# yukara-ikemiya/friendly-stable-audio-tools

Measured on NVIDIA B200. Metric: denoise_steps_per_s, higher is better.
Workload: dtype fp16 operands, fp32 accumulate (the reference's autocast dtype)

## Files before the change

### friendly-stable-audio-tools_b200/csrc/api.cu

```cuda
#include "../../include/satb200.h"
#include "common.cuh"
#include "gemm.cuh"
#include "kernels.h"

using namespace satb;

extern "C" {

int satb_snake_beta(const float* x, const float* alpha, const float* beta, float* y, int B, int C, long long T,
                    int logscale, void* stream) {
  SATB_REQUIRE(x && alpha && beta && y, "null argument");
  return launch_snake_beta(x, alpha, beta, y, B, C, T, logscale, static_cast<cudaStream_t>(stream));
}

int satb_layernorm(const float* x, const float* gamma, const float* beta, void* out16, int rows, int D, int bf16,
                   void* stream) {
  SATB_REQUIRE(x && gamma && out16, "null argument");
  return launch_layernorm(x, gamma, beta, out16, rows, D, nullptr, nullptr, 0, 1, 1, bf16 != 0,
                          static_cast<cudaStream_t>(stream));
}

int satb_linear_f32out(const void* a16, const void* w16, float* c, int M, int N, int K, int bf16, void* stream) {
  SATB_REQUIRE(a16 && w16 && c, "null argument");
  SATB_REQUIRE(M >= 1 && N >= 32 && N % 32 == 0 && K >= 8 && K % 8 == 0, "linear: need N % 32 == 0 and K % 8 == 0");
  CUtensorMap ta, tb;
  cudaStream_t st = static_cast<cudaStream_t>(stream);
  GemmShape s;
  s.L = M; s.batches = 1; s.N = N; s.K = K; s.n_taps = 1; s.tap_base = 0; s.tap_step = 0; s.b_tap_rows = N; s.stride = 1;
  EpiStore32::Params ep{c, N, nullptr};
  SATB_PROPAGATE(make_tmap_a(&ta, a16, K, M, 1, K, static_cast<int64_t>(M) * K));
  if ((N % 256 == 0 || N > 256) && gemm_use_2cta() && M >= 1024) {
    SATB_PROPAGATE(make_tmap_b(&tb, w16, K, N, K, 128));
    return bf16 ? launch_gemm_2cta<EpiStore32, 256, true>(ta, tb, s, ep, st) : launch_gemm_2cta<EpiStore32, 256, false>(ta, tb, s, ep, st);
  }
  if (N % 256 == 0 || N > 256) {
    SATB_PROPAGATE(make_tmap_b(&tb, w16, K, N, K, 256));
    return bf16 ? launch_gemm<EpiStore32, 256, true>(ta, tb, s, ep, st) : launch_gemm<EpiStore32, 256, false>(ta, tb, s, ep, st);
  } else if (N > 64) {
    SATB_PROPAGATE(make_tmap_b(&tb, w16, K, N, K, 128));
    return bf16 ? launch_gemm<EpiStore32, 128, true>(ta, tb, s, ep, st) : launch_gemm<EpiStore32, 128, false>(ta, tb, s, ep, st);
  }
  SATB_PROPAGATE(make_tmap_b(&tb, w16, K, N, K, 64));
  return bf16 ? launch_gemm<EpiStore32, 64, true>(ta, tb, s, ep, st) : launch_gemm<EpiStore32, 64, false>(ta, tb, s, ep, st);
}

int satb_sampler_update(const float* x, const float* v, const float* den_1, const float* den_2, const float* noise,
                        float* den, float* x_next, float* x_in_next, long long n, float c_skip, float c_out, float a,
                        float b, float c, float d, float s, float c_in_next, void* stream) {
  SATB_REQUIRE(x && v && den && x_next, "null argument");
  return launch_sampler_update(x, v, den_1, den_2, noise, den, x_next, x_in_next, n, c_skip, c_out, a, b, c, d, s,
                               c_in_next, static_cast<cudaStream_t>(stream));
}

int satb_attention(const void* q16, const void* k16, const void* v16, void* o16, int B, int H, int Hkv, int Nq, int Nk,
                   int bf16, void* stream) {
  SATB_REQUIRE(q16 && k16 && v16 && o16, "null argument");
  const int64_t dq = static_cast<int64_t>(H) * 64, dk = static_cast<int64_t>(Hkv) * 64;
  return launch_attention_tc(q16, k16, v16, o16, dq, dk, dk, dq, Nq * dq, Nk * dk, Nk * dk, Nq * dq, static_cast<int>(dq),
                             static_cast<int>(dk), static_cast<int>(dk), 0, 0, 0, B, H, Hkv, Nq, Nk, bf16 != 0,
                             static_cast<cudaStream_t>(stream));
}

int satb_debug_attention_occupancy(int dyn_smem, int carveout_pct) { return debug_attention_occupancy(dyn_smem, carveout_pct); }

int satb_attention_trace(const void* q16, const void* k16, const void* v16, void* o16, int B, int H, int Hkv, int Nq,
                         int Nk, int bf16, unsigned long long* dbg, void* stream) {
  const int64_t dq = static_cast<int64_t>(H) * 64, dk = static_cast<int64_t>(Hkv) * 64;
  return launch_attention_tc(q16, k16, v16, o16, dq, dk, dk, dq, Nq * dq, Nk * dk, Nk * dk, Nq * dq, static_cast<int>(dq),
                             static_cast<int>(dk), static_cast<int>(dk), 0, 0, 0, B, H, Hkv, Nq, Nk, bf16 != 0,
                             static_cast<cudaStream_t>(stream), dbg);
}

}
```

### friendly-stable-audio-tools_b200/csrc/dit.cu

```cuda
#include <cmath>
#include <cstring>
#include <map>
#include <string>
#include <tuple>
#include <vector>

#include "../../include/satb200.h"
#include "common.cuh"
#include "gemm.cuh"
#include "kernels.h"

namespace satb {

struct DevBuf {
  void* p = nullptr;
  size_t bytes = 0;
  int ensure(size_t need) {
    if (need <= bytes) return 0;
    if (p) cudaFree(p);
    p = nullptr;
    bytes = 0;
    cudaError_t e = cudaMalloc(&p, need);
    if (e != cudaSuccess) {
      set_last_error(std::string("cudaMalloc failed: ") + cudaGetErrorString(e) + " (" + std::to_string(need) + " B)");
      return -2;
    }
    bytes = need;
    return 0;
  }
  void release() {
    if (p) cudaFree(p);
    p = nullptr;
    bytes = 0;
  }
  template <class T>
  T* as() const {
    return static_cast<T*>(p);
  }
};

struct TmapCache {
  typedef std::tuple<const void*, int, int, int, int64_t, int64_t, int> Key;
  std::map<Key, CUtensorMap> maps;
  int get_a(const void* ptr, int K, int L, int batches, int64_t rs, int64_t bs, const CUtensorMap** out) {
    Key k(ptr, K, L, batches, rs, bs, -1);
    auto it = maps.find(k);
    if (it == maps.end()) {
      CUtensorMap m;
      SATB_PROPAGATE(make_tmap_a(&m, ptr, K, L, batches, rs, bs));
      it = maps.emplace(k, m).first;
    }
    *out = &it->second;
    return 0;
  }
  int get_b(const void* ptr, int K, int rows, int64_t rs, int box_rows, const CUtensorMap** out) {
    Key k(ptr, K, rows, 0, rs, 0, box_rows);
    auto it = maps.find(k);
    if (it == maps.end()) {
      CUtensorMap m;
      SATB_PROPAGATE(make_tmap_b(&m, ptr, K, rows, rs, box_rows));
      it = maps.emplace(k, m).first;
    }
    *out = &it->second;
    return 0;
  }
};

template <class Epi, int BN, bool BF16>
static int linear(TmapCache& tc, const void* A, int64_t lda, int M, int K, const void* W, int N,
                  const typename Epi::Params& ep, cudaStream_t stream) {
  const CUtensorMap *ta, *tb;
  SATB_PROPAGATE(tc.get_a(A, K, M, 1, lda, static_cast<int64_t>(M) * lda, &ta));
  GemmShape s;
  s.L = M; s.batches = 1; s.N = N; s.K = K; s.n_taps = 1; s.tap_base = 0; s.tap_step = 0; s.b_tap_rows = N; s.stride = 1;
  s.b_static = 1;
  if constexpr (BN == 256 || BN == 128) {
    if (gemm_use_2cta() && M >= 1024) {
      SATB_PROPAGATE(tc.get_b(W, K, N, K, BN / 2, &tb));
      return launch_gemm_2cta<Epi, BN, BF16>(*ta, *tb, s, ep, stream);
    }
  }
  SATB_PROPAGATE(tc.get_b(W, K, N, K, BN, &tb));
  return launch_gemm<Epi, BN, BF16>(*ta, *tb, s, ep, stream);
}

template <class Epi, bool BF16>
static int linear_auto(TmapCache& tc, const void* A, int64_t lda, int M, int K, const void* W, int N,
                       const typename Epi::Params& ep, cudaStream_t stream) {
  const double sms = device_sm_count();
  auto eff = [&](int bn) {
    const double waves = static_cast<double>(ceil_div(M, kBlockM)) * ceil_div(N, bn) / sms;
    return waves / std::ceil(waves);
  };
  if (N % 128 == 0 && eff(128) * 0.9 > eff(256)) return linear<Epi, 128, BF16>(tc, A, lda, M, K, W, N, ep, stream);
  return linear<Epi, 256, BF16>(tc, A, lda, M, K, W, N, ep, stream);
}

struct LayerW {
  float *pre_g = nullptr, *pre_b = nullptr, *ca_g = nullptr, *ca_b = nullptr, *ff_g = nullptr, *ff_b = nullptr;
  uint16_t *w_qkv = nullptr, *w_o = nullptr, *w_q = nullptr, *w_kv = nullptr, *w_co = nullptr, *w_ff1 = nullptr,
           *w_ff2 = nullptr;
  float *b_ff1 = nullptr, *b_ff2 = nullptr;
  float *c_qkv = nullptr, *d_qkv = nullptr, *c_q = nullptr, *d_q = nullptr, *c_ff1 = nullptr, *d_ff1 = nullptr;
};

}

using namespace satb;

struct SatbDit {
  SatbDitConfig cfg;
  int D, H, dh, C, Cin, ct, ce, gd, ge, ffi, depth, F, nf;
  int pdim = 0;
  float *pe0_w = nullptr, *pe2_w = nullptr;
  int Pp = 0;
  DevBuf ws_prep;
  bool bf16, adaln, qk_norm = false;
  bool ln_fused = false;
  int P;
  std::vector<LayerW> layers;
  std::vector<void*> owned;
  float *ts_w = nullptr, *te0_w = nullptr, *te0_b = nullptr, *te2_w = nullptr, *te2_b = nullptr;
  uint16_t *ce0_w = nullptr, *ce2_w = nullptr;
  float *ge0_w = nullptr, *ge2_w = nullptr;
  float *pre_w = nullptr, *post_w = nullptr, *pin_w = nullptr, *pout_w = nullptr, *inv_freq = nullptr;
  uint16_t *w_in16 = nullptr, *w_out16 = nullptr;
  float* w_ssg = nullptr;
  int* ff_perm = nullptr;
  std::map<std::string, int> loaded;
  bool finalized = false;
  int B = 0, Mctx = 0, Rc = 0;
  bool cfg_on = false, has_cross = false, has_global = false;
  TmapCache tmaps;
  DevBuf ws_h, ws_a16, ws_qkv, ws_attn, ws_q16, ws_ff, ws_ain, ws_y, ws_small, ws_cond, ws_kv, ws_rope, ws_stats;
  int rope_len = 0;
  int res_R = 0, res_L = 0, res_P = -1;
  bool prof_on = false;
  struct ProfRec { int cat; cudaEvent_t a, b; };
  std::vector<ProfRec> prof_recs;
  std::vector<cudaEvent_t> prof_pool;
  cudaEvent_t prof_event() {
    if (!prof_pool.empty()) { cudaEvent_t e = prof_pool.back(); prof_pool.pop_back(); return e; }
    cudaEvent_t e; cudaEventCreate(&e); return e;
  }

  template <class T>
  int alloc(T** p, size_t n) {
    void* q = nullptr;
    cudaError_t e = cudaMalloc(&q, n * sizeof(T) < 256 ? 256 : n * sizeof(T));
    if (e != cudaSuccess) {
      set_last_error(std::string("cudaMalloc failed: ") + cudaGetErrorString(e));
      return -2;
    }
    owned.push_back(q);
    *p = static_cast<T*>(q);
    return 0;
  }
};

static bool ends_with(const std::string& s, const std::string& suf) {
  return s.size() >= suf.size() && s.compare(s.size() - suf.size(), suf.size(), suf) == 0;
}

extern "C" {

const char* satb_last_error(void) { return get_last_error(); }
unsigned long long satb_launch_count(void) { return g_launch_count; }
void satb_reset_launch_count(void) { g_launch_count = 0; }
void satb_add_launch_count(unsigned long long n) { g_launch_count += n; }
int satb_abi_version(void) { return SATB_ABI_VERSION; }

int satb_dit_create(const SatbDitConfig* cfg, SatbDit** out) {
  SATB_REQUIRE(cfg && out, "null argument");
  SATB_REQUIRE(cfg->embed_dim % 128 == 0, "embed_dim must be a multiple of 128");
  SATB_REQUIRE(cfg->num_heads > 0 && cfg->embed_dim / cfg->num_heads == 64 && cfg->embed_dim % cfg->num_heads == 0,
               "head dim must be 64");
  SATB_REQUIRE(cfg->io_channels % 8 == 0 && cfg->io_channels % 32 == 0, "io_channels must be a multiple of 32");
  SATB_REQUIRE(cfg->patch_size == 1, "patch_size 1 only");
  SATB_REQUIRE(cfg->input_concat_dim >= 0 && cfg->input_concat_dim % 8 == 0, "input_concat_dim must be a multiple of 8");
  SATB_REQUIRE(cfg->prepend_cond_dim >= 0 && cfg->prepend_cond_dim % 4 == 0, "prepend_cond_dim must be a multiple of 4");
  SATB_REQUIRE(!(cfg->prepend_cond_dim > 0 && cfg->global_cond_type == 1),
               "prepend conditioning is supported with global_cond_type \"prepend\" only");
  SatbDit* d = new SatbDit();
  d->cfg = *cfg;
  d->D = cfg->embed_dim;
  d->H = cfg->num_heads;
  d->dh = d->D / d->H;
  d->C = cfg->io_channels;
  d->Cin = cfg->io_channels + (cfg->input_concat_dim > 0 ? cfg->input_concat_dim : 0);
  d->pdim = cfg->prepend_cond_dim > 0 ? cfg->prepend_cond_dim : 0;
  d->ct = cfg->cond_token_dim;
  d->ce = cfg->project_cond_tokens ? d->D : d->ct;
  d->gd = cfg->global_cond_dim;
  d->ge = cfg->project_global_cond ? d->D : d->gd;
  d->ffi = 4 * d->D;
  d->depth = cfg->depth;
  d->F = 128;
  const int rot = d->dh / 2 > 32 ? d->dh / 2 : 32;
  d->nf = rot / 2;
  d->bf16 = cfg->operand_dtype == 1;
  d->adaln = cfg->global_cond_type == 1;
  d->qk_norm = cfg->qk_norm != 0;
  d->P = d->adaln ? 0 : 1;
  if (d->ct > 0) {
    if (d->ce % 64 != 0 || d->H % (d->ce / 64) != 0) {
      delete d;
      set_last_error("cond embed dim must be a multiple of 64 with kv heads dividing num_heads");
      return -1;
    }
  }
  if (d->gd > 0 && d->ge != d->D) {
    delete d;
    set_last_error("global embed dim must equal embed_dim");
    return -1;
  }
  SATB_REQUIRE(d->nf == 16, "rotary dim must be 32 (head dim 64)");
  d->layers.resize(d->depth);
  *out = d;
  return 0;
}

void satb_dit_destroy(SatbDit* d) {
  if (!d) return;
  for (void* p : d->owned) cudaFree(p);
  d->ws_h.release(); d->ws_a16.release(); d->ws_qkv.release(); d->ws_attn.release(); d->ws_q16.release();
  d->ws_ff.release(); d->ws_ain.release(); d->ws_y.release(); d->ws_small.release(); d->ws_cond.release();
  d->ws_kv.release(); d->ws_rope.release(); d->ws_stats.release(); d->ws_prep.release();
  delete d;
}

int satb_dit_load_weight(SatbDit* d, const char* name_c, const float* src, long long numel, void* stream_v) {
  SATB_REQUIRE(d && name_c && src, "null argument");
  cudaStream_t st = static_cast<cudaStream_t>(stream_v);
  const std::string name(name_c);
  const int D = d->D, C = d->C, Cin = d->Cin;
  auto copy_f32 = [&](float** dst, long long expect) -> int {
    SATB_REQUIRE(numel == expect, ("bad size for " + name).c_str());
    if (!*dst) SATB_PROPAGATE(d->alloc(dst, expect));
    SATB_CHECK_CUDA(cudaMemcpyAsync(*dst, src, expect * sizeof(float), cudaMemcpyDeviceToDevice, st));
    return 0;
  };
  auto cast16 = [&](uint16_t** dst, int rows, int cols, const int* perm) -> int {
    SATB_REQUIRE(numel == static_cast<long long>(rows) * cols, ("bad size for " + name).c_str());
    if (!*dst) SATB_PROPAGATE(d->alloc(dst, static_cast<size_t>(rows) * cols));
    return launch_cast_rows(src, *dst, perm, rows, cols, cols, cols, d->bf16, st);
  };
  d->finalized = false;
  d->loaded[name] = 1;
  if (name == "timestep_features.weight") return copy_f32(&d->ts_w, d->F);
  if (name == "to_timestep_embed.0.weight") return copy_f32(&d->te0_w, static_cast<long long>(D) * 2 * d->F);
  if (name == "to_timestep_embed.0.bias") return copy_f32(&d->te0_b, D);
  if (name == "to_timestep_embed.2.weight") return copy_f32(&d->te2_w, static_cast<long long>(D) * D);
  if (name == "to_timestep_embed.2.bias") return copy_f32(&d->te2_b, D);
  if (name == "to_cond_embed.0.weight") return cast16(&d->ce0_w, d->ce, d->ct, nullptr);
  if (name == "to_cond_embed.2.weight") return cast16(&d->ce2_w, d->ce, d->ce, nullptr);
  if (name == "to_global_embed.0.weight") return copy_f32(&d->ge0_w, static_cast<long long>(d->ge) * d->gd);
  if (name == "to_global_embed.2.weight") return copy_f32(&d->ge2_w, static_cast<long long>(d->ge) * d->ge);
  if (name == "preprocess_conv.weight") return copy_f32(&d->pre_w, static_cast<long long>(Cin) * Cin);
  if (name == "to_prepend_embed.0.weight" && d->pdim > 0) return copy_f32(&d->pe0_w, static_cast<long long>(D) * d->pdim);
  if (name == "to_prepend_embed.2.weight" && d->pdim > 0) return copy_f32(&d->pe2_w, static_cast<long long>(D) * D);
  if (name == "postprocess_conv.weight") return copy_f32(&d->post_w, static_cast<long long>(C) * C);
  if (name == "transformer.project_in.weight") return copy_f32(&d->pin_w, static_cast<long long>(D) * Cin);
  if (name == "transformer.project_out.weight") return copy_f32(&d->pout_w, static_cast<long long>(C) * D);
  if (name == "transformer.rotary_pos_emb.inv_freq") return copy_f32(&d->inv_freq, d->nf);
  const std::string lp = "transformer.layers.";
  if (name.compare(0, lp.size(), lp) == 0) {
    const size_t dot = name.find('.', lp.size());
    SATB_REQUIRE(dot != std::string::npos, ("bad key " + name).c_str());
    const int li = atoi(name.substr(lp.size(), dot - lp.size()).c_str());
    SATB_REQUIRE(li >= 0 && li < d->depth, ("layer index out of range in " + name).c_str());
    LayerW& L = d->layers[li];
    const std::string k = name.substr(dot + 1);
    if (k == "pre_norm.gamma") return copy_f32(&L.pre_g, D);
    if (k == "pre_norm.beta") return copy_f32(&L.pre_b, D);
    if (k == "cross_attend_norm.gamma") return copy_f32(&L.ca_g, D);
    if (k == "cross_attend_norm.beta") return copy_f32(&L.ca_b, D);
    if (k == "ff_norm.gamma") return copy_f32(&L.ff_g, D);
    if (k == "ff_norm.beta") return copy_f32(&L.ff_b, D);
    if (k == "self_attn.to_qkv.weight") return cast16(&L.w_qkv, 3 * D, D, nullptr);
    if (k == "self_attn.to_out.weight") return cast16(&L.w_o, D, D, nullptr);
    if (k == "cross_attn.to_q.weight") return cast16(&L.w_q, D, D, nullptr);
    if (k == "cross_attn.to_kv.weight") return cast16(&L.w_kv, 2 * d->ce, d->ce, nullptr);
    if (k == "cross_attn.to_out.weight") return cast16(&L.w_co, D, D, nullptr);
    if (k == "ff.ff.0.proj.weight" || k == "ff.ff.0.proj.bias") {
      if (!d->ff_perm) {
        std::vector<int> perm(2 * d->ffi);
        for (int n = 0; n < 2 * d->ffi; ++n) {
          const int g = n / 64, w = n % 64;
          perm[n] = w < 32 ? g * 32 + w : d->ffi + g * 32 + (w - 32);
        }
        SATB_PROPAGATE(d->alloc(&d->ff_perm, perm.size()));
        SATB_CHECK_CUDA(cudaMemcpy(d->ff_perm, perm.data(), perm.size() * sizeof(int), cudaMemcpyHostToDevice));
      }
      if (ends_with(k, "weight")) return cast16(&L.w_ff1, 2 * d->ffi, D, d->ff_perm);
      SATB_REQUIRE(numel == 2 * d->ffi, ("bad size for " + name).c_str());
      if (!L.b_ff1) SATB_PROPAGATE(d->alloc(&L.b_ff1, 2 * d->ffi));
      return launch_gather_f32(src, L.b_ff1, d->ff_perm, 2 * d->ffi, st);
    }
    if (k == "ff.ff.2.weight") return cast16(&L.w_ff2, D, d->ffi, nullptr);
    if (k == "ff.ff.2.bias") return copy_f32(&L.b_ff2, D);
    if (k == "to_scale_shift_gate.1.weight") {
      SATB_REQUIRE(numel == 6LL * D * D, ("bad size for " + name).c_str());
      if (!d->w_ssg) SATB_PROPAGATE(d->alloc(&d->w_ssg, static_cast<size_t>(d->depth) * 6 * D * D));
      SATB_CHECK_CUDA(cudaMemcpyAsync(d->w_ssg + static_cast<size_t>(li) * 6 * D * D, src, numel * sizeof(float),
                                      cudaMemcpyDeviceToDevice, st));
      return 0;
    }
  }
  d->loaded.erase(name);
  set_last_error("unknown DiT weight key: " + name);
  return -4;
}

int satb_dit_finalize(SatbDit* d, void* stream_v) {
  SATB_REQUIRE(d, "null handle");
  cudaStream_t st = static_cast<cudaStream_t>(stream_v);
  const int D = d->D, C = d->C;
  SATB_REQUIRE(d->ts_w && d->te0_w && d->te0_b && d->te2_w && d->te2_b, "timestep embedding weights missing");
  SATB_REQUIRE(d->pin_w && d->pout_w && d->pre_w && d->post_w, "project_in/out or pre/post conv weights missing");
  SATB_REQUIRE(d->inv_freq, "rotary inv_freq missing");
  if (d->ct > 0) SATB_REQUIRE(d->ce0_w && d->ce2_w, "to_cond_embed weights missing");
  if (d->gd > 0) SATB_REQUIRE(d->ge0_w && d->ge2_w, "to_global_embed weights missing");
  for (int i = 0; i < d->depth; ++i) {
    const LayerW& L = d->layers[i];
    SATB_REQUIRE(L.pre_g && L.ff_g && L.w_qkv && L.w_o && L.w_ff1 && L.w_ff2, "transformer layer weights missing");
    if (d->ct > 0) SATB_REQUIRE(L.ca_g && L.w_q && L.w_kv && L.w_co, "cross-attention weights missing");
  }
  if (d->adaln) SATB_REQUIRE(d->w_ssg, "adaLN to_scale_shift_gate weights missing");
  SATB_CHECK_CUDA(cudaStreamSynchronize(st));
  const int Cin = d->Cin;
  if (d->pdim > 0) SATB_REQUIRE(d->pe0_w && d->pe2_w, "to_prepend_embed weights missing");
  std::vector<float> pin(static_cast<size_t>(D) * Cin), pout(static_cast<size_t>(C) * D), pre(Cin * Cin), post(C * C);
  SATB_CHECK_CUDA(cudaMemcpy(pin.data(), d->pin_w, pin.size() * 4, cudaMemcpyDeviceToHost));
  SATB_CHECK_CUDA(cudaMemcpy(pout.data(), d->pout_w, pout.size() * 4, cudaMemcpyDeviceToHost));
  SATB_CHECK_CUDA(cudaMemcpy(pre.data(), d->pre_w, pre.size() * 4, cudaMemcpyDeviceToHost));
  SATB_CHECK_CUDA(cudaMemcpy(post.data(), d->post_w, post.size() * 4, cudaMemcpyDeviceToHost));
  std::vector<float> fin(static_cast<size_t>(D) * Cin), fout(static_cast<size_t>(C) * D);
  for (int n = 0; n < D; ++n)
    for (int c = 0; c < Cin; ++c) {
      double acc = pin[static_cast<size_t>(n) * Cin + c];
      for (int j = 0; j < Cin; ++j) acc += static_cast<double>(pin[static_cast<size_t>(n) * Cin + j]) * pre[j * Cin + c];
      fin[static_cast<size_t>(n) * Cin + c] = static_cast<float>(acc);
    }
  for (int c = 0; c < C; ++c)
    for (int k = 0; k < D; ++k) {
      double acc = pout[static_cast<size_t>(c) * D + k];
      for (int j = 0; j < C; ++j) acc += static_cast<double>(post[c * C + j]) * pout[static_cast<size_t>(j) * D + k];
      fout[static_cast<size_t>(c) * D + k] = static_cast<float>(acc);
    }
  float *tmp_in = nullptr, *tmp_out = nullptr;
  SATB_CHECK_CUDA(cudaMalloc(&tmp_in, fin.size() * 4));
  SATB_CHECK_CUDA(cudaMalloc(&tmp_out, fout.size() * 4));
  SATB_CHECK_CUDA(cudaMemcpy(tmp_in, fin.data(), fin.size() * 4, cudaMemcpyHostToDevice));
  SATB_CHECK_CUDA(cudaMemcpy(tmp_out, fout.data(), fout.size() * 4, cudaMemcpyHostToDevice));
  if (!d->w_in16) SATB_PROPAGATE(d->alloc(&d->w_in16, fin.size()));
  if (!d->w_out16) SATB_PROPAGATE(d->alloc(&d->w_out16, fout.size()));
  int rc = launch_cast_rows(tmp_in, d->w_in16, nullptr, D, Cin, Cin, Cin, d->bf16, st);
  if (rc == 0) rc = launch_cast_rows(tmp_out, d->w_out16, nullptr, C, D, D, D, d->bf16, st);
  cudaStreamSynchronize(st);
  cudaFree(tmp_in);
  cudaFree(tmp_out);
  SATB_PROPAGATE(rc);
  d->ln_fused = !d->adaln && !d->qk_norm && ln_fold_enabled() && d->D == 6 * 256;
  if (d->ln_fused) {
    for (int i = 0; i < d->depth; ++i) {
      LayerW& L = d->layers[i];
      auto prep = [&](float** c, float** dd, const uint16_t* w, const float* g, const float* b, int rows) -> int {
        bool has_beta = false;
        if (b) {
          std::vector<float> hb(D);
          SATB_CHECK_CUDA(cudaMemcpy(hb.data(), b, D * sizeof(float), cudaMemcpyDeviceToHost));
          for (float v : hb) has_beta = has_beta || v != 0.f;
        }
        if (!*c) SATB_PROPAGATE(d->alloc(c, rows));
        float* scratch = nullptr;
        if (has_beta && !*dd) SATB_PROPAGATE(d->alloc(dd, rows));
        if (!has_beta) {
          *dd = nullptr;
          SATB_PROPAGATE(d->alloc(&scratch, rows));
        }
        return launch_ln_fold_vectors(w, g, has_beta ? b : nullptr, *c, has_beta ? *dd : scratch, rows, D, d->bf16, st);
      };
      SATB_PROPAGATE(prep(&L.c_qkv, &L.d_qkv, L.w_qkv, L.pre_g, L.pre_b, 3 * D));
      if (d->ct > 0) SATB_PROPAGATE(prep(&L.c_q, &L.d_q, L.w_q, L.ca_g, L.ca_b, D));
      SATB_PROPAGATE(prep(&L.c_ff1, &L.d_ff1, L.w_ff1, L.ff_g, L.ff_b, 2 * d->ffi));
    }
    SATB_CHECK_CUDA(cudaStreamSynchronize(st));
  }
  d->tmaps.maps.clear();
  d->finalized = true;
  return 0;
}

}

static int ensure_rope(SatbDit* d, int N_seq) {
  if (d->rope_len == N_seq) return 0;
  std::vector<float> inv(d->nf), tab(static_cast<size_t>(2) * N_seq * d->nf);
  SATB_CHECK_CUDA(cudaMemcpy(inv.data(), d->inv_freq, d->nf * 4, cudaMemcpyDeviceToHost));
  for (int p = 0; p < N_seq; ++p)
    for (int j = 0; j < d->nf; ++j) {
      const float f = static_cast<float>(p) * inv[j];
      tab[static_cast<size_t>(p) * d->nf + j] = cosf(f);
      tab[static_cast<size_t>(N_seq) * d->nf + static_cast<size_t>(p) * d->nf + j] = sinf(f);
    }
  SATB_PROPAGATE(d->ws_rope.ensure(tab.size() * 4));
  SATB_CHECK_CUDA(cudaMemcpy(d->ws_rope.p, tab.data(), tab.size() * 4, cudaMemcpyHostToDevice));
  d->rope_len = N_seq;
  return 0;
}

extern "C" {

int satb_dit_reserve(SatbDit* d, int R, int L) {
  SATB_REQUIRE(d && d->finalized, "weights not finalized");
  SATB_REQUIRE(R >= 1 && L >= 1, "bad shape");
  const int N_seq = L + d->P;
  const size_t M = static_cast<size_t>(R) * N_seq;
  const int D = d->D;
  SATB_PROPAGATE(d->ws_h.ensure(M * D * 4));
  SATB_PROPAGATE(d->ws_a16.ensure(M * D * 2));
  SATB_PROPAGATE(d->ws_qkv.ensure(M * 3 * D * 2));
  SATB_PROPAGATE(d->ws_attn.ensure(M * D * 2));
  SATB_PROPAGATE(d->ws_q16.ensure(M * D * 2));
  SATB_PROPAGATE(d->ws_ff.ensure(M * d->ffi * 2));
  SATB_PROPAGATE(d->ws_ain.ensure(M * d->Cin * 2));
  SATB_PROPAGATE(d->ws_y.ensure(M * d->C * 4));
  SATB_PROPAGATE(d->ws_stats.ensure(3 * M * kLnSlots * sizeof(float2)));
  SATB_PROPAGATE(ensure_rope(d, N_seq));
  d->tmaps.maps.clear();
  d->res_R = R;
  d->res_L = L;
  d->res_P = d->P;
  return 0;
}

}

struct SmallWs {
  float *fourier, *te_h, *tok, *ge_h, *ge, *ssg;
};
static SmallWs small_ws(SatbDit* d, int R) {
  SmallWs s;
  float* p = d->ws_small.as<float>();
  s.fourier = p; p += static_cast<size_t>(R) * 2 * d->F;
  s.te_h = p;    p += static_cast<size_t>(R) * d->D;
  s.tok = p;     p += static_cast<size_t>(R) * d->D;
  s.ge_h = p;    p += static_cast<size_t>(R) * d->D;
  s.ge = p;      p += static_cast<size_t>(R) * d->D;
  s.ssg = p;
  return s;
}

extern "C" {

int satb_dit_set_prepend_cond(SatbDit* d, const float* prepend, int B, int n_tokens, void* stream_v) {
  SATB_REQUIRE(d && d->finalized, "weights not finalized");
  cudaStream_t st = static_cast<cudaStream_t>(stream_v);
  if (!prepend || n_tokens <= 0) {
    d->Pp = 0;
    d->P = d->adaln ? 0 : 1;
    return 0;
  }
  SATB_REQUIRE(d->pdim > 0 && !d->adaln, "this model has no prepend conditioning");
  SATB_REQUIRE(B >= 1, "bad batch");
  const size_t rows = static_cast<size_t>(B) * n_tokens;
  SATB_REQUIRE(rows <= 4096, "too many prepend tokens");
  SATB_PROPAGATE(d->ws_prep.ensure(2 * rows * d->D * sizeof(float)));
  float* emb = d->ws_prep.as<float>();
  float* hid = emb + rows * d->D;
  SATB_PROPAGATE(launch_skinny_linear(prepend, d->pe0_w, nullptr, nullptr, hid, static_cast<int>(rows), d->pdim, d->D, 1, st));
  SATB_PROPAGATE(launch_skinny_linear(hid, d->pe2_w, nullptr, nullptr, emb, static_cast<int>(rows), d->D, d->D, 0, st));
  d->Pp = n_tokens;
  d->P = 1 + n_tokens;
  return 0;
}

int satb_dit_prepare_cond(SatbDit* d, const float* cross, const float* neg_cross, const float* global, int B, int Mctx,
                          int use_cfg, void* stream_v) {
  SATB_REQUIRE(d && d->finalized, "weights not finalized");
  SATB_REQUIRE(B >= 1, "bad batch");
  cudaStream_t st = static_cast<cudaStream_t>(stream_v);
  const int D = d->D;
  d->B = B;
  d->cfg_on = use_cfg != 0;
  d->has_cross = cross != nullptr && d->ct > 0;
  d->has_global = global != nullptr && d->gd > 0;
  d->Mctx = d->has_cross ? Mctx : 0;
  d->Rc = d->has_cross ? ((d->cfg_on && neg_cross) ? 2 * B : B) : 0;
  SATB_REQUIRE(!(neg_cross && !d->cfg_on), "negative conditioning requires CFG");
  SATB_PROPAGATE(d->ws_small.ensure(static_cast<size_t>(2 * B) * (2 * d->F + 4 * D + 6 * D * d->depth) * 4 + 4096));
  SmallWs sw = small_ws(d, 2 * B);
  if (d->has_global) {
    SATB_PROPAGATE(launch_skinny_linear(global, d->ge0_w, nullptr, nullptr, sw.ge_h, B, d->gd, d->ge, 1, st));
    SATB_PROPAGATE(launch_skinny_linear(sw.ge_h, d->ge2_w, nullptr, nullptr, sw.ge, B, d->ge, d->ge, 0, st));
  }
  if (d->has_cross) {
    SATB_REQUIRE(Mctx >= 1, "empty cross-attention context");
    const size_t rows = static_cast<size_t>(d->Rc) * Mctx;
    const size_t in_b = rows * d->ct * 2, mid_b = rows * d->ce * 2;
    SATB_PROPAGATE(d->ws_cond.ensure(in_b + 2 * mid_b + 1024));
    uint16_t* in16 = d->ws_cond.as<uint16_t>();
    uint16_t* mid16 = in16 + rows * d->ct;
    uint16_t* ce16 = mid16 + rows * d->ce;
    SATB_PROPAGATE(launch_cast_rows(cross, in16, nullptr, B * Mctx, d->ct, d->ct, d->ct, d->bf16, st));
    if (d->Rc == 2 * B)
      SATB_PROPAGATE(launch_cast_rows(neg_cross, in16 + static_cast<size_t>(B) * Mctx * d->ct, nullptr, B * Mctx,
                                      d->ct, d->ct, d->ct, d->bf16, st));
    SATB_PROPAGATE(d->ws_kv.ensure(static_cast<size_t>(d->depth) * rows * 2 * d->ce * 2));
    d->tmaps.maps.clear();
    const int Mr = static_cast<int>(rows);
    if (d->bf16) {
      typedef EpiStore16<true> E;
      SATB_PROPAGATE((linear<E, 128, true>(d->tmaps, in16, d->ct, Mr, d->ct, d->ce0_w, d->ce, E::Params{mid16, d->ce, nullptr, 1}, st)));
      SATB_PROPAGATE((linear<E, 128, true>(d->tmaps, mid16, d->ce, Mr, d->ce, d->ce2_w, d->ce, E::Params{ce16, d->ce, nullptr, 0}, st)));
      for (int i = 0; i < d->depth; ++i) {
        uint16_t* kv = d->ws_kv.as<uint16_t>() + static_cast<size_t>(i) * rows * 2 * d->ce;
        if (d->qk_norm) {
          typedef EpiHeadNorm16<true> EN;
          SATB_PROPAGATE((linear<EN, 128, true>(d->tmaps, ce16, d->ce, Mr, d->ce, d->layers[i].w_kv, 2 * d->ce,
                                                 EN::Params{kv, 2 * d->ce, d->ce, 0, 1, nullptr, nullptr}, st)));
        } else {
          SATB_PROPAGATE((linear<E, 128, true>(d->tmaps, ce16, d->ce, Mr, d->ce, d->layers[i].w_kv, 2 * d->ce, E::Params{kv, 2 * d->ce, nullptr, 0}, st)));
        }
      }
    } else {
      typedef EpiStore16<false> E;
      SATB_PROPAGATE((linear<E, 128, false>(d->tmaps, in16, d->ct, Mr, d->ct, d->ce0_w, d->ce, E::Params{mid16, d->ce, nullptr, 1}, st)));
      SATB_PROPAGATE((linear<E, 128, false>(d->tmaps, mid16, d->ce, Mr, d->ce, d->ce2_w, d->ce, E::Params{ce16, d->ce, nullptr, 0}, st)));
      for (int i = 0; i < d->depth; ++i) {
        uint16_t* kv = d->ws_kv.as<uint16_t>() + static_cast<size_t>(i) * rows * 2 * d->ce;
        if (d->qk_norm) {
          typedef EpiHeadNorm16<false> EN;
          SATB_PROPAGATE((linear<EN, 128, false>(d->tmaps, ce16, d->ce, Mr, d->ce, d->layers[i].w_kv, 2 * d->ce,
                                                 EN::Params{kv, 2 * d->ce, d->ce, 0, 1, nullptr, nullptr}, st)));
        } else {
          SATB_PROPAGATE((linear<E, 128, false>(d->tmaps, ce16, d->ce, Mr, d->ce, d->layers[i].w_kv, 2 * d->ce, E::Params{kv, 2 * d->ce, nullptr, 0}, st)));
        }
      }
    }
  }
  return 0;
}

}

struct ProfScope {
  SatbDit* d; int cat; cudaStream_t st; cudaEvent_t a = nullptr, b = nullptr;
  ProfScope(SatbDit* d_, int cat_, cudaStream_t st_) : d(d_), cat(cat_), st(st_) {
    if (d->prof_on) { a = d->prof_event(); b = d->prof_event(); cudaEventRecord(a, st); }
  }
  ~ProfScope() {
    if (a) { cudaEventRecord(b, st); d->prof_recs.push_back({cat, a, b}); }
  }
};
enum { PROF_FF_IN = 0, PROF_FF_OUT, PROF_QKV, PROF_ATTN_SELF, PROF_ATTN_OUT, PROF_CROSS, PROF_LN, PROF_OTHER, PROF_NCAT };

template <bool BF16>
static int dit_forward_impl(SatbDit* d, const float* x, const float* t, float* out, int B, int L, float cfg_scale,
                            float scale_phi, cudaStream_t st, float* hidden_out) {
  const int D = d->D, C = d->C, H = d->H, P = d->P;
  const int R = d->cfg_on ? 2 * B : B;
  const int N_seq = L + P;
  const int M = R * N_seq;
  const int Mc = d->Rc * N_seq;
  SmallWs sw = small_ws(d, 2 * d->B);
  float* h = d->ws_h.as<float>();
  uint16_t* a16 = d->ws_a16.as<uint16_t>();
  uint16_t* qkv = d->ws_qkv.as<uint16_t>();
  uint16_t* att = d->ws_attn.as<uint16_t>();
  uint16_t* q16 = d->ws_q16.as<uint16_t>();
  uint16_t* ff = d->ws_ff.as<uint16_t>();
  uint16_t* ain = d->ws_ain.as<uint16_t>();
  float* y = d->ws_y.as<float>();
  const float* cos_tab = d->ws_rope.as<float>();
  const float* sin_tab = cos_tab + static_cast<size_t>(N_seq) * d->nf;

  SATB_PROPAGATE(launch_fourier(t, d->ts_w, sw.fourier, B, d->F, st));
  SATB_PROPAGATE(launch_skinny_linear(sw.fourier, d->te0_w, d->te0_b, nullptr, sw.te_h, B, 2 * d->F, D, 1, st));
  SATB_PROPAGATE(launch_skinny_linear(sw.te_h, d->te2_w, d->te2_b, d->has_global ? sw.ge : nullptr, sw.tok, B, D, D,
                                      d->adaln ? 1 : 0, st));
  SATB_PROPAGATE(launch_dit_pre(x, ain, R, B, d->Cin, L, P, BF16, st));
  SATB_PROPAGATE((linear<EpiStore32, 256, BF16>(d->tmaps, ain, d->Cin, M, d->Cin, d->w_in16, D, EpiStore32::Params{h, D, nullptr}, st)));
  const int64_t ssg_ld = static_cast<int64_t>(d->depth) * 6 * D;
  if (P > 0) {
    SATB_PROPAGATE(launch_write_prepend(sw.tok, d->Pp > 0 ? d->ws_prep.as<float>() : nullptr, h, R, B, N_seq, D, d->Pp, st));
  } else {
    SATB_PROPAGATE(launch_skinny_linear(sw.tok, d->w_ssg, nullptr, nullptr, sw.ssg, B, D, d->depth * 6 * D, 0, st));
    SATB_PROPAGATE(launch_gate_sigmoid(sw.ssg, B, d->depth, D, st));
  }

  const bool fused = d->ln_fused;
  float2* S1 = d->ws_stats.as<float2>();
  float2* S2 = S1 + static_cast<size_t>(M) * kLnSlots;
  float2* S3 = S2 + static_cast<size_t>(M) * kLnSlots;
  auto fold = [&](const float2* st_, const float* c, const float* dd) {
    return LnFold{st_, c, dd, 1.0f / static_cast<float>(D), 1e-5f, kLnSlots};
  };
  const LnFold no_ln{nullptr, nullptr, nullptr, 0.f, 0.f, 0};
  for (int i = 0; i < d->depth; ++i) {
    const LayerW& W = d->layers[i];
    const float* ssg_l = d->adaln ? sw.ssg + static_cast<size_t>(i) * 6 * D : nullptr;
    if (!fused || i == 0) {
      ProfScope ps(d, PROF_LN, st);
      SATB_PROPAGATE(launch_layernorm(h, W.pre_g, W.pre_b, a16, M, D, ssg_l, ssg_l ? ssg_l + D : nullptr, ssg_ld, N_seq, B, BF16, st));
    }
    {
      ProfScope ps(d, PROF_QKV, st);
      if (d->qk_norm) {
        typedef EpiHeadNorm16<BF16> E;
        typename E::Params ep{qkv, 3 * D, 2 * D, 2 * D, N_seq, cos_tab, sin_tab};
        SATB_PROPAGATE((linear<E, 256, BF16>(d->tmaps, a16, D, M, D, W.w_qkv, 3 * D, ep, st)));
      } else {
        if (fused && i > 0) {
          typedef EpiQkvRope<BF16, true> E;
          typename E::Params ep{qkv, 3 * D, 2 * D, N_seq, cos_tab, sin_tab, fold(S1, W.c_qkv, W.d_qkv)};
          SATB_PROPAGATE((linear<E, 256, BF16>(d->tmaps, a16, D, M, D, W.w_qkv, 3 * D, ep, st)));
        } else {
          typedef EpiQkvRope<BF16> E;
          typename E::Params ep{qkv, 3 * D, 2 * D, N_seq, cos_tab, sin_tab, no_ln};
          SATB_PROPAGATE((linear<E, 256, BF16>(d->tmaps, a16, D, M, D, W.w_qkv, 3 * D, ep, st)));
        }
      }
    }
    {
      ProfScope ps(d, PROF_ATTN_SELF, st);
      const int64_t qs = static_cast<int64_t>(N_seq) * 3 * D;
      SATB_PROPAGATE(launch_attention_tc(qkv, qkv, qkv, att, 3 * D, 3 * D, 3 * D, D, qs, qs, qs,
                                         static_cast<int64_t>(N_seq) * D, 3 * D, 3 * D, 3 * D, 0, D, 2 * D, R, H, H,
                                         N_seq, N_seq, BF16, st));
    }
    {
      ProfScope ps(d, PROF_ATTN_OUT, st);
      if (fused) {
        typedef EpiResidualLN<BF16> E;
        typename E::Params ep{h, D, nullptr, a16, W.ca_g, W.ff_g, S2, S3, Mc};
        SATB_PROPAGATE((linear<E, 256, BF16>(d->tmaps, att, D, M, D, W.w_o, D, ep, st)));
      } else {
        EpiResidual::Params ep{h, D, nullptr, ssg_l ? ssg_l + 2 * D : nullptr, N_seq, static_cast<int>(ssg_ld), B};
        SATB_PROPAGATE((linear_auto<EpiResidual, BF16>(d->tmaps, att, D, M, D, W.w_o, D, ep, st)));
      }
    }
    if (Mc > 0) {
      ProfScope ps(d, PROF_CROSS, st);
      const int Hkv = d->ce / 64;
      if (!fused) SATB_PROPAGATE(launch_layernorm(h, W.ca_g, W.ca_b, a16, Mc, D, nullptr, nullptr, 0, N_seq, 1, BF16, st));
      if (d->qk_norm) {
        typedef EpiHeadNorm16<BF16> E;
        typename E::Params ep{q16, D, D, 0, N_seq, nullptr, nullptr};
        SATB_PROPAGATE((linear_auto<E, BF16>(d->tmaps, a16, D, Mc, D, W.w_q, D, ep, st)));
      } else {
        if (fused) {
          typedef EpiStore16<BF16, true> E;
          typename E::Params ep{q16, D, nullptr, 0, fold(S2, W.c_q, W.d_q)};
          SATB_PROPAGATE((linear_auto<E, BF16>(d->tmaps, a16, D, Mc, D, W.w_q, D, ep, st)));
        } else {
          typedef EpiStore16<BF16> E;
          typename E::Params ep{q16, D, nullptr, 0, no_ln};
          SATB_PROPAGATE((linear_auto<E, BF16>(d->tmaps, a16, D, Mc, D, W.w_q, D, ep, st)));
        }
      }
      const uint16_t* kv = d->ws_kv.as<uint16_t>() + static_cast<size_t>(i) * d->Rc * d->Mctx * 2 * d->ce;
      const int64_t kvs = static_cast<int64_t>(d->Mctx) * 2 * d->ce;
      SATB_PROPAGATE(launch_attention_tc(q16, kv, kv, att, D, 2 * d->ce, 2 * d->ce, D, static_cast<int64_t>(N_seq) * D,
                                         kvs, kvs, static_cast<int64_t>(N_seq) * D, D, 2 * d->ce, 2 * d->ce, 0, 0,
                                         d->ce, d->Rc, H, Hkv, N_seq, d->Mctx, BF16, st));
      if (fused) {
        typedef EpiResidualLN<BF16> E;
        typename E::Params ep{h, D, nullptr, a16, W.ff_g, W.ff_g, S3, S3, Mc};
        SATB_PROPAGATE((linear<E, 256, BF16>(d->tmaps, att, D, Mc, D, W.w_co, D, ep, st)));
      } else {
        EpiResidual::Params ep{h, D, nullptr, nullptr, N_seq, 0, 1};
        SATB_PROPAGATE((linear_auto<EpiResidual, BF16>(d->tmaps, att, D, Mc, D, W.w_co, D, ep, st)));
      }
    }
    if (!fused) {
      ProfScope ps(d, PROF_LN, st);
      SATB_PROPAGATE(launch_layernorm(h, W.ff_g, W.ff_b, a16, M, D, ssg_l ? ssg_l + 3 * D : nullptr,
                                      ssg_l ? ssg_l + 4 * D : nullptr, ssg_ld, N_seq, B, BF16, st));
    }
    {
      ProfScope ps(d, PROF_FF_IN, st);
      if (fused) {
        typedef EpiSwiglu<BF16, true> E;
        typename E::Params ep{ff, d->ffi, W.b_ff1, fold(S3, W.c_ff1, W.d_ff1)};
        SATB_PROPAGATE((linear<E, 256, BF16>(d->tmaps, a16, D, M, D, W.w_ff1, 2 * d->ffi, ep, st)));
      } else {
        typedef EpiSwiglu<BF16> E;
        typename E::Params ep{ff, d->ffi, W.b_ff1, no_ln};
        SATB_PROPAGATE((linear<E, 256, BF16>(d->tmaps, a16, D, M, D, W.w_ff1, 2 * d->ffi, ep, st)));
      }
    }
    {
      ProfScope ps(d, PROF_FF_OUT, st);
      if (fused) {
        const bool last = i + 1 == d->depth;
        typedef EpiResidualLN<BF16> E;
        typename E::Params ep{h, D, W.b_ff2, a16, last ? nullptr : d->layers[i + 1].pre_g, nullptr, last ? nullptr : S1, nullptr, M};
        SATB_PROPAGATE((linear<E, 256, BF16>(d->tmaps, ff, d->ffi, M, d->ffi, W.w_ff2, D, ep, st)));
      } else {
        EpiResidual::Params ep{h, D, W.b_ff2, ssg_l ? ssg_l + 5 * D : nullptr, N_seq, static_cast<int>(ssg_ld), B};
        SATB_PROPAGATE((linear_auto<EpiResidual, BF16>(d->tmaps, ff, d->ffi, M, d->ffi, W.w_ff2, D, ep, st)));
      }
    }
  }
  if (hidden_out)
    SATB_CHECK_CUDA(cudaMemcpyAsync(hidden_out, h, static_cast<size_t>(M) * D * 4, cudaMemcpyDeviceToDevice, st));
  if (!fused || d->depth == 0) SATB_PROPAGATE(launch_cast_rows(h, a16, nullptr, M, D, D, D, BF16, st));
  SATB_PROPAGATE((linear<EpiStore32, 64, BF16>(d->tmaps, a16, D, M, D, d->w_out16, C, EpiStore32::Params{y, C, nullptr}, st)));
  SATB_PROPAGATE(launch_dit_post(y, out, B, C, L, N_seq, P, d->cfg_on ? 1 : 0, cfg_scale, scale_phi, st));
  return 0;
}

extern "C" {

int satb_dit_forward(SatbDit* d, const float* x, const float* t, float* out, int B, int L, float cfg_scale,
                     float scale_phi, void* stream_v) {
  SATB_REQUIRE(d && d->finalized, "weights not finalized");
  SATB_REQUIRE(B == d->B, "batch size differs from satb_dit_prepare_cond");
  const int R = d->cfg_on ? 2 * B : B;
  if (R > d->res_R || L != d->res_L || d->P != d->res_P) SATB_PROPAGATE(satb_dit_reserve(d, R, L));
  cudaStream_t st = static_cast<cudaStream_t>(stream_v);
  return d->bf16 ? dit_forward_impl<true>(d, x, t, out, B, L, cfg_scale, scale_phi, st, nullptr)
                 : dit_forward_impl<false>(d, x, t, out, B, L, cfg_scale, scale_phi, st, nullptr);
}

int satb_dit_profile(SatbDit* d, int enable) {
  SATB_REQUIRE(d, "null handle");
  d->prof_on = enable != 0;
  return 0;
}
int satb_dit_profile_read(SatbDit* d, float* ms, int* count) {
  SATB_REQUIRE(d && ms && count, "null argument");
  for (int i = 0; i < PROF_NCAT; ++i) { ms[i] = 0.f; count[i] = 0; }
  for (auto& r : d->prof_recs) {
    SATB_CHECK_CUDA(cudaEventSynchronize(r.b));
    float t = 0.f;
    SATB_CHECK_CUDA(cudaEventElapsedTime(&t, r.a, r.b));
    ms[r.cat] += t;
    count[r.cat] += 1;
    d->prof_pool.push_back(r.a);
    d->prof_pool.push_back(r.b);
  }
  d->prof_recs.clear();
  return 0;
}

int satb_dit_forward_debug(SatbDit* d, const float* x, const float* t, float* out, float* hidden, int B, int L,
                           float cfg_scale, float scale_phi, void* stream_v) {
  SATB_REQUIRE(d && d->finalized, "weights not finalized");
  SATB_REQUIRE(B == d->B, "batch size differs from satb_dit_prepare_cond");
  const int R = d->cfg_on ? 2 * B : B;
  if (R > d->res_R || L != d->res_L || d->P != d->res_P) SATB_PROPAGATE(satb_dit_reserve(d, R, L));
  cudaStream_t st = static_cast<cudaStream_t>(stream_v);
  return d->bf16 ? dit_forward_impl<true>(d, x, t, out, B, L, cfg_scale, scale_phi, st, hidden)
                 : dit_forward_impl<false>(d, x, t, out, B, L, cfg_scale, scale_phi, st, hidden);
}

}
```

### friendly-stable-audio-tools_b200/csrc/gemm.cuh

```cuda
#pragma once
#include <type_traits>

#include "common.cuh"
#include "ptx.cuh"

namespace satb {

__device__ __forceinline__ int split_part(int idx, int n_parts) { return n_parts == 3 ? (idx == 2 ? 0 : idx + 1) : idx; }

struct GemmShape {
  int L;
  int batches;
  int N;
  int K;
  int n_taps;
  int tap_base;
  int tap_step;
  int b_tap_rows;
  int stride;
  int b_static = 0;
  int n_parts = 1;
  int b_part_rows = 0;
};

constexpr int kBlockM = 128;
constexpr int kBlockK = 64;
constexpr int kUmmaK = 16;
constexpr int kGemmThreads = 384;
constexpr int kSmemBudget = 220 * 1024;

constexpr int kEpiWarps = 8;
template <int BN, int kEpiStage = 0>
struct GemmCfg {
  static constexpr int kStageA = kBlockM * kBlockK * 2;
  static constexpr int kStageB = BN * kBlockK * 2;
  static constexpr int kStage = kStageA + kStageB;
  static constexpr int kAvail = kSmemBudget - 1024 - kEpiWarps * kEpiStage;
  static constexpr int kStages = kAvail / kStage > 8 ? 8 : kAvail / kStage;
  static constexpr int kTmemCols = 2 * BN < 32 ? 32 : 2 * BN;
  static constexpr int kSmemBytes = kStages * kStage + 1024  + 256  + kEpiWarps * kEpiStage;
  static_assert(BN == 64 || BN == 128 || BN == 256, "BN must be 64/128/256");
};

struct EpiCtx {
  int row;
  int l;
  int batch;
  int col0;
  bool valid;
  int l0;
  int L;
  int lane;
  float* stage;
  int n_tile;
  int half;
};

template <class E, class = void>
struct EpiHasState : std::false_type {};
template <class E>
struct EpiHasState<E, std::void_t<typename E::State>> : std::true_type {};
struct EpiNoStateHolder {
  struct State {};
};
template <class Epi>
struct EpiTile {
  using State = typename std::conditional<EpiHasState<Epi>::value, Epi, EpiNoStateHolder>::type::State;
  template <int N>
  __device__ static __forceinline__ void apply(const typename Epi::Params& p, const EpiCtx& c, const uint32_t (&r)[N], State& st) {
    if constexpr (EpiHasState<Epi>::value) Epi::apply(p, c, r, st);
    else Epi::apply(p, c, r);
  }
  __device__ static __forceinline__ void begin(const typename Epi::Params& p, const EpiCtx& c, State& st) {
    if constexpr (EpiHasState<Epi>::value) Epi::tile_begin(p, c, st);
  }
  __device__ static __forceinline__ void end(const typename Epi::Params& p, const EpiCtx& c, State& st) {
    if constexpr (EpiHasState<Epi>::value) Epi::tile_end(p, c, st);
  }
};

template <class Epi, int BN, bool BF16>
__global__ void __launch_bounds__(kGemmThreads, 1)
gemm_tcgen05_kernel(const __grid_constant__ CUtensorMap tmA, const __grid_constant__ CUtensorMap tmB,
                    const __grid_constant__ CUtensorMap tmA2, const GemmShape s, const typename Epi::Params ep) {
  using Cfg = GemmCfg<BN, Epi::kStageBytes>;
  extern __shared__ uint8_t smem_raw[];
  uint8_t* smem = reinterpret_cast<uint8_t*>((reinterpret_cast<uintptr_t>(smem_raw) + 1023) & ~uintptr_t(1023));
  uint64_t* bars = reinterpret_cast<uint64_t*>(smem + Cfg::kStages * Cfg::kStage);
  uint64_t* full_bar = bars;
  uint64_t* empty_bar = bars + Cfg::kStages;
  uint64_t* tfull_bar = bars + 2 * Cfg::kStages;
  uint64_t* tempty_bar = tfull_bar + 2;
  uint32_t* tmem_slot = reinterpret_cast<uint32_t*>(tempty_bar + 2);

  const int warp = threadIdx.x >> 5;
  const int lane = threadIdx.x & 31;

  const int m_tiles = (s.L + kBlockM - 1) / kBlockM;
  const int n_tiles = (s.N + BN - 1) / BN;
  const int tiles_per_n = m_tiles * s.batches;
  const int total_tiles = tiles_per_n * n_tiles;
  const int kb_per_tap = (s.K + kBlockK - 1) / kBlockK;
  const int kb_per_part = kb_per_tap * s.n_taps;
  const int num_kb = kb_per_part * s.n_parts;

  if (threadIdx.x == 0) {
    tma_prefetch_desc(&tmA);
    tma_prefetch_desc(&tmB);
    for (int i = 0; i < Cfg::kStages; ++i) {
      mbar_init(&full_bar[i], 1);
      mbar_init(&empty_bar[i], 1);
    }
    for (int i = 0; i < 2; ++i) {
      mbar_init(&tfull_bar[i], 1);
      mbar_init(&tempty_bar[i], 8);
    }
    fence_mbar_init();
  }
  if (warp == 2) {
    tmem_alloc(tmem_slot, Cfg::kTmemCols);
    tmem_relinquish();
  }
  tc_fence_before();
  __syncthreads();
  tc_fence_after();
  const uint32_t tmem_base = *tmem_slot;
  pdl_launch_dependents();
  const bool is_producer_warp = warp == 0;
  if (!is_producer_warp) pdl_wait();

  if (warp == 0) {
    if (elect_one()) {
      int pre = 0;
      if (s.b_static && static_cast<int>(blockIdx.x) < total_tiles) {
        pre = num_kb < Cfg::kStages ? num_kb : Cfg::kStages;
        const int n0 = (static_cast<int>(blockIdx.x) / tiles_per_n) * BN;
        for (int kb = 0; kb < pre; ++kb) {
          const int pidx = kb / kb_per_part, kbp = kb - pidx * kb_per_part;
          const int part = split_part(pidx, s.n_parts);
          const int tap = kbp / kb_per_tap;
          const int k0 = (kbp - tap * kb_per_tap) * kBlockK;
          mbar_expect_tx(&full_bar[kb], Cfg::kStage);
          tma_load_2d(smem + kb * Cfg::kStage + Cfg::kStageA, &tmB, &full_bar[kb], k0,
                      tap * s.b_tap_rows + n0 + (part == 2 ? s.b_part_rows : 0));
        }
      }
      pdl_wait();
      int stage = 0;
      uint32_t phase = 0;
      for (int tile = blockIdx.x; tile < total_tiles; tile += gridDim.x) {
        const int nt = tile / tiles_per_n;
        const int rem = tile - nt * tiles_per_n;
        const int batch = rem / m_tiles;
        const int m0 = (rem - batch * m_tiles) * kBlockM;
        const int n0 = nt * BN;
        for (int kb = 0; kb < num_kb; ++kb) {
          const int pidx = kb / kb_per_part, kbp = kb - pidx * kb_per_part;
          const int part = split_part(pidx, s.n_parts);
          const int tap = kbp / kb_per_tap;
          const int k0 = (kbp - tap * kb_per_tap) * kBlockK;
          mbar_wait(&empty_bar[stage], phase ^ 1);
          uint8_t* sa = smem + stage * Cfg::kStage;
          uint8_t* sb = sa + Cfg::kStageA;
          const bool b_done = tile == static_cast<int>(blockIdx.x) && kb < pre;
          if (!b_done) mbar_expect_tx(&full_bar[stage], Cfg::kStage);
          const int u = s.tap_base + tap * s.tap_step;
          int ph = 0, ro = u;
          if (s.stride > 1) {
            ro = (u >= 0) ? u / s.stride : -((-u + s.stride - 1) / s.stride);
            ph = u - ro * s.stride;
          }
          tma_load_4d(sa, part == 1 ? &tmA2 : &tmA, &full_bar[stage], k0, ph, m0 + ro, batch);
          if (!b_done)
            tma_load_2d(sb, &tmB, &full_bar[stage], k0, tap * s.b_tap_rows + n0 + (part == 2 ? s.b_part_rows : 0));
          if (++stage == Cfg::kStages) {
            stage = 0;
            phase ^= 1;
          }
        }
      }
    }
  } else if (warp == 1) {
    if (elect_one()) {
      constexpr uint32_t idesc = make_idesc_f16(kBlockM, BN, BF16);
      int stage = 0;
      uint32_t phase = 0;
      int acc = 0;
      uint32_t acc_phase = 0;
      for (int tile = blockIdx.x; tile < total_tiles; tile += gridDim.x) {
        mbar_wait(&tempty_bar[acc], acc_phase ^ 1);
        tc_fence_after();
        const uint32_t d_tmem = tmem_base + acc * BN;
        for (int kb = 0; kb < num_kb; ++kb) {
          mbar_wait(&full_bar[stage], phase);
          tc_fence_after();
          const uint32_t a_addr = smem_u32(smem + stage * Cfg::kStage);
          const uint32_t b_addr = a_addr + Cfg::kStageA;
#pragma unroll
          for (int k = 0; k < kBlockK / kUmmaK; ++k) {
            const uint64_t da = make_desc_kmajor_sw128(a_addr + k * kUmmaK * 2);
            const uint64_t db = make_desc_kmajor_sw128(b_addr + k * kUmmaK * 2);
            umma_f16_ss(d_tmem, da, db, idesc, (kb | k) != 0 ? 1u : 0u);
          }
          umma_commit(&empty_bar[stage]);
          if (++stage == Cfg::kStages) {
            stage = 0;
            phase ^= 1;
          }
        }
        umma_commit(&tfull_bar[acc]);
        if (++acc == 2) {
          acc = 0;
          acc_phase ^= 1;
        }
      }
    }
  } else if (warp >= 4) {
    const int q = warp & 3;
    const int half = (warp - 4) >> 2;
    constexpr int kChunks = BN / Epi::kCols;
    int acc = 0;
    uint32_t acc_phase = 0;
    for (int tile = blockIdx.x; tile < total_tiles; tile += gridDim.x) {
      const int nt = tile / tiles_per_n;
      const int rem = tile - nt * tiles_per_n;
      const int batch = rem / m_tiles;
      const int m0 = (rem - batch * m_tiles) * kBlockM;
      const int n0 = nt * BN;
      mbar_wait(&tfull_bar[acc], acc_phase);
      tc_fence_after();
      EpiCtx c;
      c.l = m0 + q * 32 + lane;
      c.batch = batch;
      c.row = batch * s.L + c.l;
      c.valid = c.l < s.L;
      c.l0 = m0 + q * 32;
      c.L = s.L;
      c.lane = lane;
      c.n_tile = nt;
      c.half = half;
      c.stage = Epi::kStageBytes > 0
                    ? reinterpret_cast<float*>(smem + Cfg::kStages * Cfg::kStage + 256 + (warp - 4) * Epi::kStageBytes)
                    : nullptr;
      const uint32_t t_row = tmem_base + (static_cast<uint32_t>(q * 32) << 16) + acc * BN;
      int n_valid = (s.N - n0 + Epi::kCols - 1) / Epi::kCols;
      if (n_valid > kChunks) n_valid = kChunks;
      uint32_t r0[Epi::kCols], r1[Epi::kCols];
      auto load_chunk = [&](int ci, uint32_t (&dst)[Epi::kCols]) {
#pragma unroll
        for (int j = 0; j < Epi::kCols / 32; ++j) {
          uint32_t(&rj)[32] = *reinterpret_cast<uint32_t(*)[32]>(&dst[j * 32]);
          tmem_ld_32x32(t_row + ci * Epi::kCols + j * 32, rj);
        }
      };
      typename EpiTile<Epi>::State est;
      EpiTile<Epi>::begin(ep, c, est);
      if (half < n_valid) {
        load_chunk(half, r0);
        tmem_ld_wait();
      }
#pragma unroll 1
      for (int ci = half; ci < n_valid; ci += 4) {
        const bool has1 = ci + 2 < n_valid;
        if (has1) load_chunk(ci + 2, r1);
        c.col0 = n0 + ci * Epi::kCols;
        EpiTile<Epi>::apply(ep, c, r0, est);
        tmem_ld_wait();
        if (has1) {
          if (ci + 4 < n_valid) load_chunk(ci + 4, r0);
          c.col0 = n0 + (ci + 2) * Epi::kCols;
          EpiTile<Epi>::apply(ep, c, r1, est);
          tmem_ld_wait();
        }
      }
      EpiTile<Epi>::end(ep, c, est);
      tc_fence_before();
      __syncwarp();
      if (lane == 0) mbar_arrive(&tempty_bar[acc]);
      if (++acc == 2) {
        acc = 0;
        acc_phase ^= 1;
      }
    }
  }
  tc_fence_before();
  __syncthreads();
  if (warp == 2) {
    tc_fence_after();
    tmem_dealloc(tmem_base, Cfg::kTmemCols);
  }
}

template <int BN, int kEpiStage = 0>
struct Gemm2Cfg {
  static constexpr int kStageA = kBlockM * kBlockK * 2;
  static constexpr int kStageB = (BN / 2) * kBlockK * 2;
  static constexpr int kStage = kStageA + kStageB;
  static constexpr int kAvail = kSmemBudget - 1024 - kEpiWarps * kEpiStage;
  static constexpr int kStages = kAvail / kStage > 8 ? 8 : kAvail / kStage;
  static constexpr int kTmemCols = 2 * BN;
  static constexpr int kSmemBytes = kStages * kStage + 1024 + 256 + kEpiWarps * kEpiStage;
  static_assert(BN == 256 || BN == 128, "BN must be 128/256");
};

template <class Epi, int BN, bool BF16>
__global__ void __cluster_dims__(2, 1, 1) __launch_bounds__(kGemmThreads, 1)
gemm_tcgen05_2cta_kernel(const __grid_constant__ CUtensorMap tmA, const __grid_constant__ CUtensorMap tmB,
                         const __grid_constant__ CUtensorMap tmA2, const GemmShape s, const typename Epi::Params ep) {
  using Cfg = Gemm2Cfg<BN, Epi::kStageBytes>;
  extern __shared__ uint8_t smem_raw[];
  uint8_t* smem = reinterpret_cast<uint8_t*>((reinterpret_cast<uintptr_t>(smem_raw) + 1023) & ~uintptr_t(1023));
  uint64_t* bars = reinterpret_cast<uint64_t*>(smem + Cfg::kStages * Cfg::kStage);
  uint64_t* full_bar = bars;
  uint64_t* empty_bar = bars + Cfg::kStages;
  uint64_t* tfull_bar = bars + 2 * Cfg::kStages;
  uint64_t* tempty_bar = tfull_bar + 2;
  uint32_t* tmem_slot = reinterpret_cast<uint32_t*>(tempty_bar + 2);

  const int warp = threadIdx.x >> 5;
  const int lane = threadIdx.x & 31;
  const uint32_t rank = cluster_ctarank();
  const int cluster_id = blockIdx.x >> 1, n_clusters = gridDim.x >> 1;

  const int m_tiles = (s.L + 2 * kBlockM - 1) / (2 * kBlockM);
  const int n_tiles = (s.N + BN - 1) / BN;
  const int tiles_per_n = m_tiles * s.batches;
  const int total_tiles = tiles_per_n * n_tiles;
  const int kb_per_tap = (s.K + kBlockK - 1) / kBlockK;
  const int kb_per_part = kb_per_tap * s.n_taps;
  const int num_kb = kb_per_part * s.n_parts;

  if (threadIdx.x == 0) {
    tma_prefetch_desc(&tmA);
    tma_prefetch_desc(&tmB);
    for (int i = 0; i < Cfg::kStages; ++i) {
      mbar_init(&full_bar[i], 1);
      mbar_init(&empty_bar[i], 1);
    }
    for (int i = 0; i < 2; ++i) {
      mbar_init(&tfull_bar[i], 1);
      mbar_init(&tempty_bar[i], 16);
    }
    fence_mbar_init();
  }
  cluster_sync_all();
  if (warp == 2) {
    tmem_alloc_2sm(tmem_slot, Cfg::kTmemCols);
    tmem_relinquish_2sm();
  }
  tc_fence_before();
  __syncthreads();
  tc_fence_after();
  const uint32_t tmem_base = *tmem_slot;
  pdl_launch_dependents();
  if (warp != 0) pdl_wait();

  if (warp == 0) {
    if (elect_one()) {
      int pre = 0;
      if (s.b_static && cluster_id < total_tiles) {
        pre = num_kb < Cfg::kStages ? num_kb : Cfg::kStages;
        const int n0 = (cluster_id / tiles_per_n) * BN + rank * (BN / 2);
        for (int kb = 0; kb < pre; ++kb) {
          const int pidx = kb / kb_per_part, kbp = kb - pidx * kb_per_part;
          const int part = split_part(pidx, s.n_parts);
          const int tap = kbp / kb_per_tap;
          const int k0 = (kbp - tap * kb_per_tap) * kBlockK;
          if (rank == 0) mbar_expect_tx(&full_bar[kb], 2 * Cfg::kStage);
          tma_load_2d_2sm(smem + kb * Cfg::kStage + Cfg::kStageA, &tmB, &full_bar[kb], k0,
                          tap * s.b_tap_rows + n0 + (part == 2 ? s.b_part_rows : 0));
        }
      }
      pdl_wait();
      int stage = 0;
      uint32_t phase = 0;
      for (int tile = cluster_id; tile < total_tiles; tile += n_clusters) {
        const int nt = tile / tiles_per_n;
        const int rem = tile - nt * tiles_per_n;
        const int batch = rem / m_tiles;
        const int m0 = (rem - batch * m_tiles) * 2 * kBlockM + rank * kBlockM;
        const int n0 = nt * BN + rank * (BN / 2);
        for (int kb = 0; kb < num_kb; ++kb) {
          const int pidx = kb / kb_per_part, kbp = kb - pidx * kb_per_part;
          const int part = split_part(pidx, s.n_parts);
          const int tap = kbp / kb_per_tap;
          const int k0 = (kbp - tap * kb_per_tap) * kBlockK;
          mbar_wait(&empty_bar[stage], phase ^ 1);
          uint8_t* sa = smem + stage * Cfg::kStage;
          uint8_t* sb = sa + Cfg::kStageA;
          const bool b_done = tile == cluster_id && kb < pre;
          if (rank == 0 && !b_done) mbar_expect_tx(&full_bar[stage], 2 * Cfg::kStage);
          const int u = s.tap_base + tap * s.tap_step;
          int ph = 0, ro = u;
          if (s.stride > 1) {
            ro = (u >= 0) ? u / s.stride : -((-u + s.stride - 1) / s.stride);
            ph = u - ro * s.stride;
          }
          tma_load_4d_2sm(sa, part == 1 ? &tmA2 : &tmA, &full_bar[stage], k0, ph, m0 + ro, batch);
          if (!b_done)
            tma_load_2d_2sm(sb, &tmB, &full_bar[stage], k0, tap * s.b_tap_rows + n0 + (part == 2 ? s.b_part_rows : 0));
          if (++stage == Cfg::kStages) {
            stage = 0;
            phase ^= 1;
          }
        }
      }
    }
  } else if (warp == 1) {
    if (rank == 0 && elect_one()) {
      constexpr uint32_t idesc = make_idesc_f16(2 * kBlockM, BN, BF16);
      int stage = 0;
      uint32_t phase = 0;
      int acc = 0;
      uint32_t acc_phase = 0;
      for (int tile = cluster_id; tile < total_tiles; tile += n_clusters) {
        mbar_wait(&tempty_bar[acc], acc_phase ^ 1);
        tc_fence_after();
        const uint32_t d_tmem = tmem_base + acc * BN;
        for (int kb = 0; kb < num_kb; ++kb) {
          mbar_wait(&full_bar[stage], phase);
          tc_fence_after();
          const uint32_t a_addr = smem_u32(smem + stage * Cfg::kStage);
          const uint32_t b_addr = a_addr + Cfg::kStageA;
#pragma unroll
          for (int k = 0; k < kBlockK / kUmmaK; ++k) {
            const uint64_t da = make_desc_kmajor_sw128(a_addr + k * kUmmaK * 2);
            const uint64_t db = make_desc_kmajor_sw128(b_addr + k * kUmmaK * 2);
            umma_f16_ss_2sm(d_tmem, da, db, idesc, (kb | k) != 0 ? 1u : 0u);
          }
          umma_commit_2sm(&empty_bar[stage]);
          if (++stage == Cfg::kStages) {
            stage = 0;
            phase ^= 1;
          }
        }
        umma_commit_2sm(&tfull_bar[acc]);
        if (++acc == 2) {
          acc = 0;
          acc_phase ^= 1;
        }
      }
    }
  } else if (warp >= 4) {
    const int q = warp & 3;
    const int half = (warp - 4) >> 2;
    constexpr int kChunks = BN / Epi::kCols;
    int acc = 0;
    uint32_t acc_phase = 0;
    for (int tile = cluster_id; tile < total_tiles; tile += n_clusters) {
      const int nt = tile / tiles_per_n;
      const int rem = tile - nt * tiles_per_n;
      const int batch = rem / m_tiles;
      const int m0 = (rem - batch * m_tiles) * 2 * kBlockM + rank * kBlockM;
      const int n0 = nt * BN;
      mbar_wait(&tfull_bar[acc], acc_phase);
      tc_fence_after();
      EpiCtx c;
      c.l = m0 + q * 32 + lane;
      c.batch = batch;
      c.row = batch * s.L + c.l;
      c.valid = c.l < s.L;
      c.l0 = m0 + q * 32;
      c.L = s.L;
      c.lane = lane;
      c.n_tile = nt;
      c.half = half;
      c.stage = Epi::kStageBytes > 0
                    ? reinterpret_cast<float*>(smem + Cfg::kStages * Cfg::kStage + 256 + (warp - 4) * Epi::kStageBytes)
                    : nullptr;
      const uint32_t t_row = tmem_base + (static_cast<uint32_t>(q * 32) << 16) + acc * BN;
      int n_valid = (s.N - n0 + Epi::kCols - 1) / Epi::kCols;
      if (n_valid > kChunks) n_valid = kChunks;
      uint32_t r0[Epi::kCols], r1[Epi::kCols];
      auto load_chunk = [&](int ci, uint32_t (&dst)[Epi::kCols]) {
#pragma unroll
        for (int j = 0; j < Epi::kCols / 32; ++j) {
          uint32_t(&rj)[32] = *reinterpret_cast<uint32_t(*)[32]>(&dst[j * 32]);
          tmem_ld_32x32(t_row + ci * Epi::kCols + j * 32, rj);
        }
      };
      typename EpiTile<Epi>::State est;
      EpiTile<Epi>::begin(ep, c, est);
      if (half < n_valid) {
        load_chunk(half, r0);
        tmem_ld_wait();
      }
#pragma unroll 1
      for (int ci = half; ci < n_valid; ci += 4) {
        const bool has1 = ci + 2 < n_valid;
        if (has1) load_chunk(ci + 2, r1);
        c.col0 = n0 + ci * Epi::kCols;
        EpiTile<Epi>::apply(ep, c, r0, est);
        tmem_ld_wait();
        if (has1) {
          if (ci + 4 < n_valid) load_chunk(ci + 4, r0);
          c.col0 = n0 + (ci + 2) * Epi::kCols;
          EpiTile<Epi>::apply(ep, c, r1, est);
          tmem_ld_wait();
        }
      }
      EpiTile<Epi>::end(ep, c, est);
      tc_fence_before();
      __syncwarp();
      if (lane == 0) mbar_arrive_remote(&tempty_bar[acc], 0);
      if (++acc == 2) {
        acc = 0;
        acc_phase ^= 1;
      }
    }
  }
  tc_fence_before();
  cluster_sync_all();
  if (warp == 2) {
    tc_fence_after();
    tmem_dealloc_2sm(tmem_base, Cfg::kTmemCols);
  }
}


constexpr int kLnSlots = 12;
struct LnFold {
  const float2* stats;
  const float* c;
  const float* d;
  float inv_dim;
  float eps;
  int n_slots;
};
struct LnRow {
  float rstd, mr;
};
__device__ __forceinline__ LnRow ln_row(const LnFold& f, int row) {
  const float4* sp = reinterpret_cast<const float4*>(f.stats + static_cast<size_t>(row) * kLnSlots);
  float s1 = 0.f, s2 = 0.f;
#pragma unroll
  for (int i = 0; i < kLnSlots / 2; ++i) {
    if (2 * i < f.n_slots) {
      const float4 v = __ldg(sp + i);
      s1 += v.x + v.z;
      s2 += v.y + v.w;
    }
  }
  const float mean = s1 * f.inv_dim;
  const float var = fmaxf(s2 * f.inv_dim - mean * mean, 0.f);
  LnRow r;
  r.rstd = rsqrtf(var + f.eps);
  r.mr = mean * r.rstd;
  return r;
}
__device__ __forceinline__ void ln_apply4(const LnFold& f, const LnRow& r, float& v0, float& v1, float& v2, float& v3, int col) {
  const float4 cc = __ldg(reinterpret_cast<const float4*>(f.c + col));
  v0 = fmaf(v0, r.rstd, -r.mr * cc.x);
  v1 = fmaf(v1, r.rstd, -r.mr * cc.y);
  v2 = fmaf(v2, r.rstd, -r.mr * cc.z);
  v3 = fmaf(v3, r.rstd, -r.mr * cc.w);
  if (f.d) {
    const float4 dd = __ldg(reinterpret_cast<const float4*>(f.d + col));
    v0 += dd.x; v1 += dd.y; v2 += dd.z; v3 += dd.w;
  }
}

__device__ __forceinline__ float silu_f(float x) { return x / (1.0f + __expf(-x)); }

template <bool BF16, bool LN = false>
struct EpiStore16 {
  static constexpr int kCols = 32;
  static constexpr int kStageBytes = 0;
  struct Params {
    void* out;
    int ld;
    const float* bias;
    int act;
    LnFold ln = LnFold{nullptr, nullptr, nullptr, 0.f, 0.f, 0};
  };
  __device__ static __forceinline__ void apply(const Params& p, const EpiCtx& c, const uint32_t (&r)[32]) {
    if (!c.valid) return;
    float v[32];
#pragma unroll
    for (int j = 0; j < 32; ++j) v[j] = __uint_as_float(r[j]);
    if constexpr (LN) {
      const LnRow lr = ln_row(p.ln, c.row);
#pragma unroll
      for (int j = 0; j < 32; j += 4) ln_apply4(p.ln, lr, v[j], v[j + 1], v[j + 2], v[j + 3], c.col0 + j);
    }
    if (p.bias) {
#pragma unroll
      for (int j = 0; j < 32; j += 4) {
        const float4 b = __ldg(reinterpret_cast<const float4*>(p.bias + c.col0 + j));
        v[j] += b.x; v[j + 1] += b.y; v[j + 2] += b.z; v[j + 3] += b.w;
      }
    }
    uint32_t o[16];
#pragma unroll
    for (int j = 0; j < 16; ++j) {
      float a = v[2 * j], b = v[2 * j + 1];
      if (p.act == 1) {
        a = silu_f(a);
        b = silu_f(b);
      }
      o[j] = Op16<BF16>::pack(a, b);
    }
    uint4* dst = reinterpret_cast<uint4*>(static_cast<uint16_t*>(p.out) + static_cast<size_t>(c.row) * p.ld + c.col0);
#pragma unroll
    for (int j = 0; j < 4; ++j) dst[j] = make_uint4(o[4 * j], o[4 * j + 1], o[4 * j + 2], o[4 * j + 3]);
  }
};

struct EpiStore32 {
  static constexpr int kCols = 32;
  static constexpr int kStageBytes = 0;
  struct Params {
    float* out;
    int ld;
    const float* bias;
  };
  __device__ static __forceinline__ void apply(const Params& p, const EpiCtx& c, const uint32_t (&r)[32]) {
    if (!c.valid) return;
    float4* dst = reinterpret_cast<float4*>(p.out + static_cast<size_t>(c.row) * p.ld + c.col0);
#pragma unroll
    for (int j = 0; j < 8; ++j) {
      float4 v = make_float4(__uint_as_float(r[4 * j]), __uint_as_float(r[4 * j + 1]), __uint_as_float(r[4 * j + 2]),
                             __uint_as_float(r[4 * j + 3]));
      if (p.bias) {
        const float4 b = __ldg(reinterpret_cast<const float4*>(p.bias + c.col0) + j);
        v.x += b.x; v.y += b.y; v.z += b.z; v.w += b.w;
      }
      dst[j] = v;
    }
  }
};

struct EpiResidual {
  static constexpr int kCols = 32;
  static constexpr int kStageBytes = 0;
  struct Params {
    float* h;
    int ld;
    const float* bias;
    const float* gate;
    int rows_per_item;
    int gate_ld;
    int n_items;
  };
  __device__ static __forceinline__ void apply(const Params& p, const EpiCtx& c, const uint32_t (&r)[32]) {
    if (!c.valid) return;
    float4* dst = reinterpret_cast<float4*>(p.h + static_cast<size_t>(c.row) * p.ld + c.col0);
    const float4* g = p.gate ? reinterpret_cast<const float4*>(
                                   p.gate + static_cast<size_t>((c.row / p.rows_per_item) % p.n_items) * p.gate_ld + c.col0)
                             : nullptr;
#pragma unroll
    for (int j = 0; j < 8; ++j) {
      float4 v = make_float4(__uint_as_float(r[4 * j]), __uint_as_float(r[4 * j + 1]), __uint_as_float(r[4 * j + 2]),
                             __uint_as_float(r[4 * j + 3]));
      if (p.bias) {
        const float4 b = __ldg(reinterpret_cast<const float4*>(p.bias + c.col0) + j);
        v.x += b.x; v.y += b.y; v.z += b.z; v.w += b.w;
      }
      if (g) {
        const float4 gg = __ldg(g + j);
        v.x *= gg.x; v.y *= gg.y; v.z *= gg.z; v.w *= gg.w;
      }
      asm volatile("red.global.add.v4.f32 [%0], {%1, %2, %3, %4};" ::"l"(dst + j), "f"(v.x), "f"(v.y), "f"(v.z), "f"(v.w)
                   : "memory");
    }
  }
};

template <bool BF16>
struct EpiResidualLN {
  static constexpr int kCols = 32;
  static constexpr int kStageBytes = 32 * 36 * 4;
  struct Params {
    float* h;
    int ld;
    const float* bias;
    void* x16;
    const float* gamma_lo;
    const float* gamma_hi;
    float2* stats_lo;
    float2* stats_hi;
    int split;
  };
  struct State {
    float s1[8], s2[8];
  };
  __device__ static __forceinline__ void tile_begin(const Params&, const EpiCtx&, State& st) {
#pragma unroll
    for (int i = 0; i < 8; ++i) st.s1[i] = st.s2[i] = 0.f;
  }
  __device__ static __forceinline__ void apply(const Params& p, const EpiCtx& c, const uint32_t (&r)[32], State& st) {
    const int g = c.lane & 7, r0 = c.lane >> 3;
    const int col = c.col0 + 4 * g;
    float4 old[8];
#pragma unroll
    for (int i = 0; i < 8; ++i) {
      const int l = c.l0 + r0 + 4 * i;
      old[i] = l < c.L ? *reinterpret_cast<const float4*>(p.h + (static_cast<size_t>(c.batch) * c.L + l) * p.ld + col)
                       : make_float4(0.f, 0.f, 0.f, 0.f);
    }
    float* stg = c.stage;
    {
      float4* mine = reinterpret_cast<float4*>(stg + c.lane * 36);
#pragma unroll
      for (int j = 0; j < 8; ++j)
        mine[j] = make_float4(__uint_as_float(r[4 * j]), __uint_as_float(r[4 * j + 1]), __uint_as_float(r[4 * j + 2]),
                              __uint_as_float(r[4 * j + 3]));
    }
    __syncwarp();
    float4 b4 = make_float4(0.f, 0.f, 0.f, 0.f), glo = make_float4(1.f, 1.f, 1.f, 1.f), ghi = glo;
    if (p.bias) b4 = __ldg(reinterpret_cast<const float4*>(p.bias + col));
    if (p.gamma_lo) glo = __ldg(reinterpret_cast<const float4*>(p.gamma_lo + col));
    if (p.gamma_hi) ghi = __ldg(reinterpret_cast<const float4*>(p.gamma_hi + col));
#pragma unroll
    for (int i = 0; i < 8; ++i) {
      const int l = c.l0 + r0 + 4 * i;
      if (l < c.L) {
        const size_t row = static_cast<size_t>(c.batch) * c.L + l;
        const float4 a = *reinterpret_cast<const float4*>(stg + (r0 + 4 * i) * 36 + 4 * g);
        float4 v;
        v.x = a.x + b4.x + old[i].x; v.y = a.y + b4.y + old[i].y; v.z = a.z + b4.z + old[i].z; v.w = a.w + b4.w + old[i].w;
        *reinterpret_cast<float4*>(p.h + row * p.ld + col) = v;
        st.s1[i] += (v.x + v.y) + (v.z + v.w);
        st.s2[i] = fmaf(v.x, v.x, fmaf(v.y, v.y, fmaf(v.z, v.z, fmaf(v.w, v.w, st.s2[i]))));
        const float4 gg = static_cast<int>(row) < p.split ? glo : ghi;
        *reinterpret_cast<uint2*>(static_cast<uint16_t*>(p.x16) + row * p.ld + col) =
            make_uint2(Op16<BF16>::pack(v.x * gg.x, v.y * gg.y), Op16<BF16>::pack(v.z * gg.z, v.w * gg.w));
      }
    }
    __syncwarp();
  }
  __device__ static __forceinline__ void tile_end(const Params& p, const EpiCtx& c, State& st) {
    const int g = c.lane & 7, r0 = c.lane >> 3;
    const int slot = c.n_tile * 2 + c.half;
#pragma unroll
    for (int i = 0; i < 8; ++i) {
      float a = st.s1[i], b = st.s2[i];
#pragma unroll
      for (int o = 1; o < 8; o <<= 1) {
        a += __shfl_xor_sync(0xffffffffu, a, o);
        b += __shfl_xor_sync(0xffffffffu, b, o);
      }
      const int l = c.l0 + r0 + 4 * i;
      if (g == 0 && l < c.L && slot < kLnSlots) {
        const size_t row = static_cast<size_t>(c.batch) * c.L + l;
        float2* sp = static_cast<int>(row) < p.split ? p.stats_lo : p.stats_hi;
        if (sp) sp[row * kLnSlots + slot] = make_float2(a, b);
      }
    }
  }
};

template <bool BF16, bool LN = false>
struct EpiQkvRope {
  static constexpr int kCols = 32;
  static constexpr int kStageBytes = 0;
  struct Params {
    void* out;
    int ld;
    int rope_cols;
    int seq_len;
    const float* cos_tab;
    const float* sin_tab;
    LnFold ln = LnFold{nullptr, nullptr, nullptr, 0.f, 0.f, 0};
  };
  __device__ static __forceinline__ void apply(const Params& p, const EpiCtx& c, const uint32_t (&r)[32]) {
    if (!c.valid) return;
    float v[32];
#pragma unroll
    for (int j = 0; j < 32; ++j) v[j] = __uint_as_float(r[j]);
    if constexpr (LN) {
      const LnRow lr = ln_row(p.ln, c.row);
#pragma unroll
      for (int j = 0; j < 32; j += 4) ln_apply4(p.ln, lr, v[j], v[j + 1], v[j + 2], v[j + 3], c.col0 + j);
    }
    if (c.col0 < p.rope_cols && ((c.col0 >> 5) & 1) == 0 && p.cos_tab) {
      const int pos = c.row % p.seq_len;
      const float4* ct = reinterpret_cast<const float4*>(p.cos_tab + pos * 16);
      const float4* st = reinterpret_cast<const float4*>(p.sin_tab + pos * 16);
#pragma unroll
      for (int j4 = 0; j4 < 4; ++j4) {
        const float4 cs = __ldg(ct + j4), sn = __ldg(st + j4);
        const float cc[4] = {cs.x, cs.y, cs.z, cs.w}, ss[4] = {sn.x, sn.y, sn.z, sn.w};
#pragma unroll
        for (int u = 0; u < 4; ++u) {
          const int j = j4 * 4 + u;
          const float a = v[j], b = v[j + 16];
          v[j] = a * cc[u] - b * ss[u];
          v[j + 16] = b * cc[u] + a * ss[u];
        }
      }
    }
    uint4* dst = reinterpret_cast<uint4*>(static_cast<uint16_t*>(p.out) + static_cast<size_t>(c.row) * p.ld + c.col0);
#pragma unroll
    for (int j = 0; j < 4; ++j)
      dst[j] = make_uint4(Op16<BF16>::pack(v[8 * j], v[8 * j + 1]), Op16<BF16>::pack(v[8 * j + 2], v[8 * j + 3]),
                          Op16<BF16>::pack(v[8 * j + 4], v[8 * j + 5]), Op16<BF16>::pack(v[8 * j + 6], v[8 * j + 7]));
  }
};

template <bool BF16>
struct EpiHeadNorm16 {
  static constexpr int kCols = 64;
  static constexpr int kStageBytes = 0;
  struct Params {
    void* out;
    int ld;
    int norm_cols;
    int rope_cols;
    int seq_len;
    const float* cos_tab;
    const float* sin_tab;
  };
  __device__ static __forceinline__ void apply(const Params& p, const EpiCtx& c, const uint32_t (&r)[64]) {
    if (!c.valid) return;
    float inv = 1.f;
    if (c.col0 < p.norm_cols) {
      float ss = 0.f;
#pragma unroll
      for (int j = 0; j < 64; ++j) ss = fmaf(__uint_as_float(r[j]), __uint_as_float(r[j]), ss);
      inv = 1.f / fmaxf(sqrtf(ss), 1e-12f);
    }
    uint4* dst = reinterpret_cast<uint4*>(static_cast<uint16_t*>(p.out) + static_cast<size_t>(c.row) * p.ld + c.col0);
    float v[32];
#pragma unroll
    for (int j = 0; j < 32; ++j) v[j] = __uint_as_float(r[j]) * inv;
    if (c.col0 < p.rope_cols && p.cos_tab) {
      const int pos = c.row % p.seq_len;
      const float4* ct = reinterpret_cast<const float4*>(p.cos_tab + pos * 16);
      const float4* st = reinterpret_cast<const float4*>(p.sin_tab + pos * 16);
#pragma unroll
      for (int j4 = 0; j4 < 4; ++j4) {
        const float4 cs = __ldg(ct + j4), sn = __ldg(st + j4);
        const float cc[4] = {cs.x, cs.y, cs.z, cs.w}, ss4[4] = {sn.x, sn.y, sn.z, sn.w};
#pragma unroll
        for (int u = 0; u < 4; ++u) {
          const int j = j4 * 4 + u;
          const float a = v[j], b = v[j + 16];
          v[j] = a * cc[u] - b * ss4[u];
          v[j + 16] = b * cc[u] + a * ss4[u];
        }
      }
    }
#pragma unroll
    for (int j = 0; j < 4; ++j)
      dst[j] = make_uint4(Op16<BF16>::pack(v[8 * j], v[8 * j + 1]), Op16<BF16>::pack(v[8 * j + 2], v[8 * j + 3]),
                          Op16<BF16>::pack(v[8 * j + 4], v[8 * j + 5]), Op16<BF16>::pack(v[8 * j + 6], v[8 * j + 7]));
#pragma unroll
    for (int j = 0; j < 4; ++j) {
      const uint32_t* q = &r[32 + 8 * j];
      dst[4 + j] = make_uint4(Op16<BF16>::pack(__uint_as_float(q[0]) * inv, __uint_as_float(q[1]) * inv),
                              Op16<BF16>::pack(__uint_as_float(q[2]) * inv, __uint_as_float(q[3]) * inv),
                              Op16<BF16>::pack(__uint_as_float(q[4]) * inv, __uint_as_float(q[5]) * inv),
                              Op16<BF16>::pack(__uint_as_float(q[6]) * inv, __uint_as_float(q[7]) * inv));
    }
  }
};

template <bool BF16, bool LN = false>
struct EpiSwiglu {
  static constexpr int kCols = 64;
  static constexpr int kStageBytes = 0;
  struct Params {
    void* out;
    int ld;
    const float* bias;
    LnFold ln = LnFold{nullptr, nullptr, nullptr, 0.f, 0.f, 0};
  };
  __device__ static __forceinline__ void apply(const Params& p, const EpiCtx& c, const uint32_t (&r)[64]) {
    if (!c.valid) return;
    uint32_t o[16];
    if constexpr (!LN) {
#pragma unroll
      for (int j = 0; j < 16; ++j) {
        float a0 = __uint_as_float(r[2 * j]), a1 = __uint_as_float(r[2 * j + 1]);
        float g0 = __uint_as_float(r[32 + 2 * j]), g1 = __uint_as_float(r[33 + 2 * j]);
        if (p.bias) {
          a0 += __ldg(p.bias + c.col0 + 2 * j);
          a1 += __ldg(p.bias + c.col0 + 2 * j + 1);
          g0 += __ldg(p.bias + c.col0 + 32 + 2 * j);
          g1 += __ldg(p.bias + c.col0 + 33 + 2 * j);
        }
        o[j] = Op16<BF16>::pack(a0 * silu_f(g0), a1 * silu_f(g1));
      }
      uint4* dst0 =
          reinterpret_cast<uint4*>(static_cast<uint16_t*>(p.out) + static_cast<size_t>(c.row) * p.ld + (c.col0 >> 1));
#pragma unroll
      for (int j = 0; j < 4; ++j) dst0[j] = make_uint4(o[4 * j], o[4 * j + 1], o[4 * j + 2], o[4 * j + 3]);
      return;
    }
    LnRow lr{1.f, 0.f};
    if constexpr (LN) lr = ln_row(p.ln, c.row);
#pragma unroll
    for (int j = 0; j < 8; ++j) {
      float a0 = __uint_as_float(r[4 * j]), a1 = __uint_as_float(r[4 * j + 1]), a2 = __uint_as_float(r[4 * j + 2]),
            a3 = __uint_as_float(r[4 * j + 3]);
      float g0 = __uint_as_float(r[32 + 4 * j]), g1 = __uint_as_float(r[33 + 4 * j]), g2 = __uint_as_float(r[34 + 4 * j]),
            g3 = __uint_as_float(r[35 + 4 * j]);
      if constexpr (LN) {
        ln_apply4(p.ln, lr, a0, a1, a2, a3, c.col0 + 4 * j);
        ln_apply4(p.ln, lr, g0, g1, g2, g3, c.col0 + 32 + 4 * j);
      }
      if (p.bias) {
        const float4 ba = __ldg(reinterpret_cast<const float4*>(p.bias + c.col0 + 4 * j));
        const float4 bg = __ldg(reinterpret_cast<const float4*>(p.bias + c.col0 + 32 + 4 * j));
        a0 += ba.x; a1 += ba.y; a2 += ba.z; a3 += ba.w;
        g0 += bg.x; g1 += bg.y; g2 += bg.z; g3 += bg.w;
      }
      o[2 * j] = Op16<BF16>::pack(a0 * silu_f(g0), a1 * silu_f(g1));
      o[2 * j + 1] = Op16<BF16>::pack(a2 * silu_f(g2), a3 * silu_f(g3));
    }
    uint4* dst =
        reinterpret_cast<uint4*>(static_cast<uint16_t*>(p.out) + static_cast<size_t>(c.row) * p.ld + (c.col0 >> 1));
#pragma unroll
    for (int j = 0; j < 4; ++j) dst[j] = make_uint4(o[4 * j], o[4 * j + 1], o[4 * j + 2], o[4 * j + 3]);
  }
};

__device__ __forceinline__ float snake_fast(float v, float a, float ib) {
  const float sn = __sinf(v * a);
  return fmaf(ib, sn * sn, v);
}

__device__ __forceinline__ uint64_t f2_pack(float lo, float hi) {
  uint64_t d;
  asm("mov.b64 %0, {%1, %2};" : "=l"(d) : "f"(lo), "f"(hi));
  return d;
}
__device__ __forceinline__ void f2_unpack(uint64_t v, float& lo, float& hi) {
  asm("mov.b64 {%0, %1}, %2;" : "=f"(lo), "=f"(hi) : "l"(v));
}
__device__ __forceinline__ uint64_t f2_add(uint64_t a, uint64_t b) {
  uint64_t d;
  asm("add.rn.f32x2 %0, %1, %2;" : "=l"(d) : "l"(a), "l"(b));
  return d;
}
__device__ __forceinline__ uint64_t f2_mul(uint64_t a, uint64_t b) {
  uint64_t d;
  asm("mul.rn.f32x2 %0, %1, %2;" : "=l"(d) : "l"(a), "l"(b));
  return d;
}
__device__ __forceinline__ uint64_t f2_fma(uint64_t a, uint64_t b, uint64_t c) {
  uint64_t d;
  asm("fma.rn.f32x2 %0, %1, %2, %3;" : "=l"(d) : "l"(a), "l"(b), "l"(c));
  return d;
}
__device__ __forceinline__ uint64_t snake_fast2(uint64_t v, uint64_t a, uint64_t ib) {
  float t0, t1;
  f2_unpack(f2_mul(v, a), t0, t1);
  const uint64_t sn = f2_pack(__sinf(t0), __sinf(t1));
  return f2_fma(ib, f2_mul(sn, sn), v);
}

struct EpiConvParams {
  const float* bias;
  const void* resid;
  void* raw_out;
  void* s16_out;
  const float* sn_a;
  const float* sn_ib;
  int cout;
  int L_out;
  int up;
  int pad;
  void* s16_lo_out;
  int raw16;
};
template <bool BF16, bool MASKED = false>
struct EpiConv {
  static constexpr int kCols = 32;
  static constexpr int kStageBytes = 32 * 36 * 4;
  typedef EpiConvParams Params;
  __host__ __device__ static bool fast_flags(const Params& p) {
    return p.s16_out != nullptr && p.sn_a != nullptr && p.s16_lo_out == nullptr &&
           (p.raw16 != 0 || (p.resid == nullptr && p.raw_out == nullptr));
  }
  struct Seg {
    int phase, co;
  };
  __device__ static __forceinline__ Seg seg_of(const Params& p, const EpiCtx& c) {
    Seg sg{0, c.col0};
    if (p.up > 1) {
      sg.phase = c.col0 / p.cout;
      sg.co = c.col0 - sg.phase * p.cout;
    }
    sg.co += 4 * (c.lane & 7);
    return sg;
  }
  __device__ static __forceinline__ bool seg_index(const Params& p, const EpiCtx& c, const Seg& sg, int i, size_t* idx) {
    const int l = c.l0 + (c.lane >> 3) + 4 * i;
    const int lo = l * p.up + sg.phase - p.pad;
    const bool ok = l < c.L && lo >= 0 && lo < p.L_out;
    *idx = (static_cast<size_t>(c.batch) * p.L_out + (ok ? lo : 0)) * p.cout + sg.co;
    return ok;
  }
  struct Plan {
    size_t idx0;
    int stride;
    bool fast;
    int co;
  };
  __device__ static __forceinline__ Plan plan_of(const Params& p, const EpiCtx& c) {
    const Seg sg = seg_of(p, c);
    const int l_first = c.l0 + (c.lane >> 3), l_last = l_first + 28;
    const int lo_first = l_first * p.up + sg.phase - p.pad, lo_last = l_last * p.up + sg.phase - p.pad;
    const bool ok = l_last < c.L && lo_first >= 0 && lo_last < p.L_out;
    const bool flags = fast_flags(p);
    Plan pl;
    pl.fast = flags && __all_sync(0xffffffffu, ok);
    pl.idx0 = (static_cast<size_t>(c.batch) * p.L_out + (ok ? lo_first : 0)) * p.cout + sg.co;
    pl.stride = 4 * p.up * p.cout;
    pl.co = sg.co;
    return pl;
  }
  template <bool RESID, bool RAWOUT, bool SNAKE>
  __device__ static __forceinline__ void finish_fast(const Params& p, const EpiCtx& c, const Plan& pl, const uint32_t (&r)[32],
                                                     const float4 (&rs)[8]) {
    const uint32_t st = smem_u32(c.stage);
    const int g = c.lane & 7, r0 = c.lane >> 3;
#pragma unroll
    for (int j = 0; j < 8; ++j) sts128(st + (c.lane * 36 + 4 * j) * 4, r[4 * j], r[4 * j + 1], r[4 * j + 2], r[4 * j + 3]);
    __syncwarp();
    ulonglong2 b2 = make_ulonglong2(0ull, 0ull), a2 = b2, ib2 = b2;
    if (p.bias) b2 = __ldg(reinterpret_cast<const ulonglong2*>(p.bias + pl.co));
    if (SNAKE) {
      a2 = __ldg(reinterpret_cast<const ulonglong2*>(p.sn_a + pl.co));
      ib2 = __ldg(reinterpret_cast<const ulonglong2*>(p.sn_ib + pl.co));
    }
    uint16_t* raw_o = static_cast<uint16_t*>(p.raw_out) + pl.idx0;
    uint16_t* s_o = static_cast<uint16_t*>(p.s16_out) + pl.idx0;
    uint32_t ld_addr = st + (r0 * 36 + 4 * g) * 4;
#pragma unroll
    for (int i = 0; i < 8; ++i) {
      const ulonglong2 acc = lds128_b64x2(ld_addr);
      ld_addr += 4 * 36 * 4;
      uint64_t v01 = f2_add(acc.x, b2.x), v23 = f2_add(acc.y, b2.y);
      if (RESID) {
        const float2 lo = Op16<BF16>::unpack(__float_as_uint(rs[i].x)), hi = Op16<BF16>::unpack(__float_as_uint(rs[i].y));
        v01 = f2_add(v01, f2_pack(lo.x, lo.y));
        v23 = f2_add(v23, f2_pack(hi.x, hi.y));
      }
      if (RAWOUT) {
        float y0, y1, y2, y3;
        f2_unpack(v01, y0, y1);
        f2_unpack(v23, y2, y3);
        *reinterpret_cast<uint2*>(raw_o) = make_uint2(Op16<BF16>::pack(y0, y1), Op16<BF16>::pack(y2, y3));
        raw_o += pl.stride;
      }
      if (SNAKE) {
        v01 = snake_fast2(v01, a2.x, ib2.x);
        v23 = snake_fast2(v23, a2.y, ib2.y);
      }
      float x0, x1, x2, x3;
      f2_unpack(v01, x0, x1);
      f2_unpack(v23, x2, x3);
      *reinterpret_cast<uint2*>(s_o) = make_uint2(Op16<BF16>::pack(x0, x1), Op16<BF16>::pack(x2, x3));
      s_o += pl.stride;
    }
    __syncwarp();
  }
  struct MPlan {
    long long idx0;
    int stride;
    uint32_t mask;
    int co;
  };
  __device__ static __forceinline__ MPlan mplan_of(const Params& p, const EpiCtx& c) {
    const Seg sg = seg_of(p, c);
    const int l0 = c.l0 + (c.lane >> 3);
    const int lo0 = l0 * p.up + sg.phase - p.pad;
    MPlan pl;
    pl.mask = 0;
#pragma unroll
    for (int i = 0; i < 8; ++i) {
      const int l = l0 + 4 * i, lo = lo0 + 4 * i * p.up;
      if (l < c.L && lo >= 0 && lo < p.L_out) pl.mask |= 1u << i;
    }
    pl.idx0 = (static_cast<long long>(c.batch) * p.L_out + lo0) * p.cout + sg.co;
    pl.stride = 4 * p.up * p.cout;
    pl.co = sg.co;
    return pl;
  }
  __device__ static __forceinline__ void prefetch_masked(const Params& p, const EpiCtx& c, float4 (&rs)[8]) {
    if (p.resid) {
      const MPlan pl = mplan_of(p, c);
      const uint16_t* rp = static_cast<const uint16_t*>(p.resid) + pl.idx0;
#pragma unroll
      for (int i = 0; i < 8; ++i) {
        uint2 u = make_uint2(0u, 0u);
        if ((pl.mask >> i) & 1u) u = *reinterpret_cast<const uint2*>(rp);
        rp += pl.stride;
        rs[i] = make_float4(__uint_as_float(u.x), __uint_as_float(u.y), 0.f, 0.f);
      }
    }
  }
  template <bool RESID, bool RAWOUT>
  __device__ static __forceinline__ void finish_masked_t(const Params& p, const EpiCtx& c, const uint32_t (&r)[32],
                                                         const float4 (&rs)[8]) {
    const MPlan pl = mplan_of(p, c);
    const uint32_t st = smem_u32(c.stage);
    const int g = c.lane & 7, r0 = c.lane >> 3;
#pragma unroll
    for (int j = 0; j < 8; ++j) sts128(st + (c.lane * 36 + 4 * j) * 4, r[4 * j], r[4 * j + 1], r[4 * j + 2], r[4 * j + 3]);
    __syncwarp();
    ulonglong2 b2 = make_ulonglong2(0ull, 0ull);
    if (p.bias) b2 = __ldg(reinterpret_cast<const ulonglong2*>(p.bias + pl.co));
    const ulonglong2 a2 = __ldg(reinterpret_cast<const ulonglong2*>(p.sn_a + pl.co));
    const ulonglong2 ib2 = __ldg(reinterpret_cast<const ulonglong2*>(p.sn_ib + pl.co));
    uint16_t* raw_o = static_cast<uint16_t*>(p.raw_out) + pl.idx0;
    uint16_t* s_o = static_cast<uint16_t*>(p.s16_out) + pl.idx0;
    uint32_t ld_addr = st + (r0 * 36 + 4 * g) * 4;
#pragma unroll
    for (int i = 0; i < 8; ++i) {
      const ulonglong2 acc = lds128_b64x2(ld_addr);
      ld_addr += 4 * 36 * 4;
      const bool ok = (pl.mask >> i) & 1u;
      uint64_t v01 = f2_add(acc.x, b2.x), v23 = f2_add(acc.y, b2.y);
      if (RESID) {
        const float2 lo = Op16<BF16>::unpack(__float_as_uint(rs[i].x)), hi = Op16<BF16>::unpack(__float_as_uint(rs[i].y));
        v01 = f2_add(v01, f2_pack(lo.x, lo.y));
        v23 = f2_add(v23, f2_pack(hi.x, hi.y));
      }
      if (RAWOUT) {
        float y0, y1, y2, y3;
        f2_unpack(v01, y0, y1);
        f2_unpack(v23, y2, y3);
        if (ok) *reinterpret_cast<uint2*>(raw_o) = make_uint2(Op16<BF16>::pack(y0, y1), Op16<BF16>::pack(y2, y3));
        raw_o += pl.stride;
      }
      v01 = snake_fast2(v01, a2.x, ib2.x);
      v23 = snake_fast2(v23, a2.y, ib2.y);
      float x0, x1, x2, x3;
      f2_unpack(v01, x0, x1);
      f2_unpack(v23, x2, x3);
      if (ok) *reinterpret_cast<uint2*>(s_o) = make_uint2(Op16<BF16>::pack(x0, x1), Op16<BF16>::pack(x2, x3));
      s_o += pl.stride;
    }
    __syncwarp();
  }
  __device__ static __forceinline__ void finish_masked(const Params& p, const EpiCtx& c, const uint32_t (&r)[32],
                                                       const float4 (&rs)[8]) {
    if (p.resid) {
      if (p.raw_out) finish_masked_t<true, true>(p, c, r, rs);
      else finish_masked_t<true, false>(p, c, r, rs);
    } else {
      if (p.raw_out) finish_masked_t<false, true>(p, c, r, rs);
      else finish_masked_t<false, false>(p, c, r, rs);
    }
  }
  __device__ static __forceinline__ void prefetch(const Params& p, const EpiCtx& c, float4 (&rs)[8]) {
    if constexpr (MASKED) {
      prefetch_masked(p, c, rs);
      return;
    }
    {
      const Plan pl = plan_of(p, c);
      if (pl.fast) {
        if (p.resid) {
          const uint16_t* rp = static_cast<const uint16_t*>(p.resid) + pl.idx0;
#pragma unroll
          for (int i = 0; i < 8; ++i) {
            const uint2 u = *reinterpret_cast<const uint2*>(rp);
            rp += pl.stride;
            rs[i] = make_float4(__uint_as_float(u.x), __uint_as_float(u.y), 0.f, 0.f);
          }
        }
        return;
      }
    }
    const Seg sg = seg_of(p, c);
#pragma unroll
    for (int i = 0; i < 8; ++i) {
      size_t idx;
      const bool ok = seg_index(p, c, sg, i, &idx);
      rs[i] = make_float4(0.f, 0.f, 0.f, 0.f);
      if (ok && p.resid) {
        if (p.raw16) {
          const uint2 u = *reinterpret_cast<const uint2*>(static_cast<const uint16_t*>(p.resid) + idx);
          rs[i] = make_float4(__uint_as_float(u.x), __uint_as_float(u.y), 0.f, 0.f);
        } else {
          rs[i] = *reinterpret_cast<const float4*>(static_cast<const float*>(p.resid) + idx);
        }
      }
    }
  }
  __device__ static __forceinline__ void finish(const Params& p, const EpiCtx& c, const uint32_t (&r)[32],
                                                const float4 (&rs)[8]) {
    if constexpr (MASKED) {
      finish_masked(p, c, r, rs);
      return;
    }
    {
      const Plan pl = plan_of(p, c);
      if (pl.fast) {
        if (p.resid) {
          if (p.raw_out) finish_fast<true, true, true>(p, c, pl, r, rs);
          else finish_fast<true, false, true>(p, c, pl, r, rs);
        } else {
          if (p.raw_out) finish_fast<false, true, true>(p, c, pl, r, rs);
          else finish_fast<false, false, true>(p, c, pl, r, rs);
        }
        return;
      }
    }
    float* st = c.stage;
    const int g = c.lane & 7, r0 = c.lane >> 3;
    {
      float4* mine = reinterpret_cast<float4*>(st + c.lane * 36);
#pragma unroll
      for (int j = 0; j < 8; ++j)
        mine[j] = make_float4(__uint_as_float(r[4 * j]), __uint_as_float(r[4 * j + 1]), __uint_as_float(r[4 * j + 2]),
                              __uint_as_float(r[4 * j + 3]));
    }
    __syncwarp();
    const Seg sg = seg_of(p, c);
    const int co = sg.co;
    ulonglong2 b2 = make_ulonglong2(0ull, 0ull), a2 = b2, ib2 = b2;
    if (p.bias) b2 = __ldg(reinterpret_cast<const ulonglong2*>(p.bias + co));
    const bool snake = p.s16_out != nullptr && p.sn_a != nullptr;
    if (snake) {
      a2 = __ldg(reinterpret_cast<const ulonglong2*>(p.sn_a + co));
      ib2 = __ldg(reinterpret_cast<const ulonglong2*>(p.sn_ib + co));
    }
#pragma unroll
    for (int i = 0; i < 8; ++i) {
      size_t idx;
      if (seg_index(p, c, sg, i, &idx)) {
        const ulonglong2 acc = *reinterpret_cast<const ulonglong2*>(st + (r0 + 4 * i) * 36 + 4 * g);
        uint64_t r01, r23;
        if (p.raw16 && p.resid) {
          const float2 lo = Op16<BF16>::unpack(__float_as_uint(rs[i].x)), hi = Op16<BF16>::unpack(__float_as_uint(rs[i].y));
          r01 = f2_pack(lo.x, lo.y);
          r23 = f2_pack(hi.x, hi.y);
        } else {
          r01 = f2_pack(rs[i].x, rs[i].y);
          r23 = f2_pack(rs[i].z, rs[i].w);
        }
        uint64_t v01 = f2_add(acc.x, f2_add(b2.x, r01));
        uint64_t v23 = f2_add(acc.y, f2_add(b2.y, r23));
        if (p.raw_out) {
          if (p.raw16) {
            float y0, y1, y2, y3;
            f2_unpack(v01, y0, y1);
            f2_unpack(v23, y2, y3);
            *reinterpret_cast<uint2*>(static_cast<uint16_t*>(p.raw_out) + idx) =
                make_uint2(Op16<BF16>::pack(y0, y1), Op16<BF16>::pack(y2, y3));
          } else {
            *reinterpret_cast<ulonglong2*>(static_cast<float*>(p.raw_out) + idx) = make_ulonglong2(v01, v23);
          }
        }
        if (p.s16_out) {
          if (snake) {
            v01 = snake_fast2(v01, a2.x, ib2.x);
            v23 = snake_fast2(v23, a2.y, ib2.y);
          }
          float x0, x1, x2, x3;
          f2_unpack(v01, x0, x1);
          f2_unpack(v23, x2, x3);
          const uint32_t h01 = Op16<BF16>::pack(x0, x1), h23 = Op16<BF16>::pack(x2, x3);
          *reinterpret_cast<uint2*>(static_cast<uint16_t*>(p.s16_out) + idx) = make_uint2(h01, h23);
          if (p.s16_lo_out) {
            const float2 a = Op16<BF16>::unpack(h01), b = Op16<BF16>::unpack(h23);
            *reinterpret_cast<uint2*>(static_cast<uint16_t*>(p.s16_lo_out) + idx) =
                make_uint2(Op16<BF16>::pack(x0 - a.x, x1 - a.y), Op16<BF16>::pack(x2 - b.x, x3 - b.y));
          }
        }
      }
    }
    __syncwarp();
  }
  __device__ static __forceinline__ void apply(const Params& p, const EpiCtx& c, const uint32_t (&r)[32]) {
    float4 rs[8];
    prefetch(p, c, rs);
    finish(p, c, r, rs);
  }
};

struct EpiStoreNCL {
  static constexpr int kCols = 32;
  static constexpr int kStageBytes = 0;
  struct Params {
    float* out;
    const float* bias;
    int N;
    int L;
    int do_tanh;
  };
  __device__ static __forceinline__ void apply(const Params& p, const EpiCtx& c, const uint32_t (&r)[32]) {
    if (!c.valid) return;
    float* o = p.out + (static_cast<size_t>(c.batch) * p.N + c.col0) * p.L + c.l;
#pragma unroll
    for (int j = 0; j < 32; ++j) {
      if (c.col0 + j < p.N) {
        const float v = __uint_as_float(r[j]) + (p.bias ? __ldg(p.bias + c.col0 + j) : 0.f);
        o[static_cast<size_t>(j) * p.L] = p.do_tanh ? tanhf(v) : v;
      }
    }
  }
};

int make_tmap_a(CUtensorMap* m, const void* ptr, int K, int L, int batches, int64_t row_stride_elems,
                int64_t batch_stride_elems, int stride = 1, int box_rows = kBlockM);
int make_tmap_b(CUtensorMap* m, const void* ptr, int K, int rows, int64_t row_stride_elems, int box_rows);

template <class Epi, int BN, bool BF16>
int launch_gemm(const CUtensorMap& tmA, const CUtensorMap& tmB, const GemmShape& s, const typename Epi::Params& ep,
                cudaStream_t stream, const CUtensorMap* tmA2 = nullptr) {
  using Cfg = GemmCfg<BN, Epi::kStageBytes>;
  auto kern = gemm_tcgen05_kernel<Epi, BN, BF16>;
  static PerDeviceOnce attr;
  if (attr.first()) SATB_CHECK_CUDA(cudaFuncSetAttribute(kern, cudaFuncAttributeMaxDynamicSharedMemorySize, Cfg::kSmemBytes));
  const int m_tiles = ceil_div(s.L, kBlockM), n_tiles = ceil_div(s.N, BN);
  const int total = m_tiles * s.batches * n_tiles;
  if (total <= 0) return 0;
  int grid = device_sm_count();
  if (grid > total) grid = total;
  SATB_REQUIRE(s.n_parts == 1 || tmA2 != nullptr, "split-operand GEMM needs the second A tensor map");
  SATB_CHECK_CUDA(launch_pdl(kern, dim3(grid), dim3(kGemmThreads), Cfg::kSmemBytes, stream, tmA, tmB, tmA2 ? *tmA2 : tmA, s, ep));
  count_launch();
  return 0;
}

template <class Epi, int BN, bool BF16>
int launch_gemm_2cta(const CUtensorMap& tmA, const CUtensorMap& tmB, const GemmShape& s, const typename Epi::Params& ep,
                     cudaStream_t stream, const CUtensorMap* tmA2 = nullptr) {
  using Cfg = Gemm2Cfg<BN, Epi::kStageBytes>;
  auto kern = gemm_tcgen05_2cta_kernel<Epi, BN, BF16>;
  static PerDeviceOnce attr;
  if (attr.first()) SATB_CHECK_CUDA(cudaFuncSetAttribute(kern, cudaFuncAttributeMaxDynamicSharedMemorySize, Cfg::kSmemBytes));
  const int m_tiles = ceil_div(s.L, 2 * kBlockM), n_tiles = ceil_div(s.N, BN);
  const int total = m_tiles * s.batches * n_tiles;
  if (total <= 0) return 0;
  int clusters = device_sm_count() / 2;
  if (clusters > total) clusters = total;
  SATB_REQUIRE(s.n_parts == 1 || tmA2 != nullptr, "split-operand GEMM needs the second A tensor map");
  SATB_CHECK_CUDA(launch_pdl(kern, dim3(2 * clusters), dim3(kGemmThreads), Cfg::kSmemBytes, stream, tmA, tmB,
                             tmA2 ? *tmA2 : tmA, s, ep));
  count_launch();
  return 0;
}

}
```

### friendly-stable-audio-tools_b200/csrc/kernels.h

```cpp
#pragma once
#include <cuda_runtime.h>
#include <stdint.h>

namespace satb {

int launch_attention_tc(const void* q, const void* k, const void* v, void* o, int64_t ldq, int64_t ldk, int64_t ldv,
                        int64_t ldo, int64_t q_bs, int64_t k_bs, int64_t v_bs, int64_t o_bs, int q_cols, int k_cols,
                        int v_cols, int q_col, int k_col, int v_col, int batch, int H, int H_kv, int Nq, int Nk,
                        bool bf16, cudaStream_t stream, unsigned long long* dbg = nullptr);
int debug_attention_occupancy(int dyn_smem, int carveout_pct);
bool conv_halo_enabled();
bool conv_epi_masked();
bool resunit_use_fused();
bool gemm_use_2cta();
bool ln_fold_enabled();
bool raw_stream_16bit();

int launch_layernorm(const float* x, const float* gamma, const float* beta, void* out16, int rows, int D,
                     const float* scale, const float* shift, int64_t mod_stride, int rows_per_item, int n_items,
                     bool bf16, cudaStream_t stream);
int launch_ln_fold_vectors(const void* w16, const float* gamma, const float* beta, float* c, float* d, int rows, int K,
                           bool bf16, cudaStream_t stream);
int launch_sampler_update(const float* x, const float* v, const float* d1, const float* d2, const float* nz, float* den,
                          float* x_next, float* x_in, long long n, float c_skip, float c_out, float A, float B, float C,
                          float D, float S, float c_in_next, cudaStream_t stream);
int launch_snake_beta(const float* x, const float* alpha, const float* beta, float* y, int B, int C, int64_t T,
                      int logscale, cudaStream_t stream);
int launch_dit_pre(const float* x, void* a16, int R, int B_src, int C, int L, int P, bool bf16, cudaStream_t stream);
int launch_fourier(const float* t, const float* w, float* out, int B, int F, cudaStream_t stream);
int launch_skinny_linear(const float* in, const float* W, const float* bias, const float* add, float* out, int R,
                         int K, int N, int silu_out, cudaStream_t stream);
int launch_write_prepend(const float* tok, const float* pre, float* h, int R, int B, int N_seq, int D, int Pp,
                         cudaStream_t stream);
int launch_gate_sigmoid(float* ssg, int rows, int depth, int D, cudaStream_t stream);
int launch_dit_post(const float* y, float* out, int B, int C, int L, int N_seq, int P, int cfg, float cfg_scale,
                    float scale_phi, cudaStream_t stream);
int launch_cast_rows(const float* src, void* dst, const int* perm, int rows, int cols, int64_t src_ld, int64_t dst_ld,
                     bool bf16, cudaStream_t stream);
int launch_gather_f32(const float* src, float* dst, const int* perm, int n, cudaStream_t stream);
int launch_zero(void* p, size_t bytes, cudaStream_t stream);

}
```

### friendly-stable-audio-tools_b200/csrc/ptx.cuh

```cuda
#pragma once
#include <cuda.h>
#include <cuda_runtime.h>
#include <stdint.h>

namespace satb {

__device__ __forceinline__ uint32_t smem_u32(const void* p) {
  return static_cast<uint32_t>(__cvta_generic_to_shared(p));
}

__device__ __forceinline__ bool elect_one() {
  uint32_t pred = 0;
  asm volatile(
      "{\n\t.reg .pred P;\n\t"
      "elect.sync _|P, 0xffffffff;\n\t"
      "selp.u32 %0, 1, 0, P;\n\t}"
      : "=r"(pred));
  return pred != 0;
}

__device__ __forceinline__ void pdl_wait() { asm volatile("griddepcontrol.wait;" ::: "memory"); }
__device__ __forceinline__ void pdl_launch_dependents() { asm volatile("griddepcontrol.launch_dependents;" ::: "memory"); }

__device__ __forceinline__ void mbar_init(uint64_t* bar, uint32_t count) {
  asm volatile("mbarrier.init.shared::cta.b64 [%0], %1;" ::"r"(smem_u32(bar)), "r"(count));
}
__device__ __forceinline__ void fence_mbar_init() {
  asm volatile("fence.mbarrier_init.release.cluster;" ::: "memory");
}
__device__ __forceinline__ void fence_proxy_async_smem() {
  asm volatile("fence.proxy.async.shared::cta;" ::: "memory");
}
__device__ __forceinline__ void mbar_expect_tx(uint64_t* bar, uint32_t bytes) {
  asm volatile("mbarrier.arrive.expect_tx.shared::cta.b64 _, [%0], %1;" ::"r"(smem_u32(bar)), "r"(bytes)
               : "memory");
}
__device__ __forceinline__ void mbar_arrive(uint64_t* bar) {
  asm volatile("mbarrier.arrive.shared::cta.b64 _, [%0];" ::"r"(smem_u32(bar)) : "memory");
}
constexpr uint32_t kMbarSuspendHintNs = 20000;
__device__ __forceinline__ bool mbar_try_wait(uint64_t* bar, uint32_t parity) {
  uint32_t ok;
  asm volatile(
      "{\n\t.reg .pred P;\n\t"
      "mbarrier.try_wait.parity.shared::cta.b64 P, [%1], %2, %3;\n\t"
      "selp.u32 %0, 1, 0, P;\n\t}"
      : "=r"(ok)
      : "r"(smem_u32(bar)), "r"(parity), "r"(kMbarSuspendHintNs)
      : "memory");
  return ok != 0;
}
__device__ __forceinline__ void mbar_spin(uint64_t* bar, uint32_t parity) {
  uint32_t ok;
  do {
    asm volatile(
        "{\n\t.reg .pred P;\n\t"
        "mbarrier.test_wait.parity.shared::cta.b64 P, [%1], %2;\n\t"
        "selp.u32 %0, 1, 0, P;\n\t}"
        : "=r"(ok)
        : "r"(smem_u32(bar)), "r"(parity)
        : "memory");
  } while (!ok);
}
__device__ __forceinline__ void mbar_wait(uint64_t* bar, uint32_t parity) {
  while (!mbar_try_wait(bar, parity)) {
  }
}

__device__ __forceinline__ void tma_prefetch_desc(const CUtensorMap* m) {
  asm volatile("prefetch.tensormap [%0];" ::"l"(reinterpret_cast<uint64_t>(m)) : "memory");
}
__device__ __forceinline__ void tma_load_2d(void* smem, const CUtensorMap* m, uint64_t* bar, int c0, int c1) {
  asm volatile(
      "cp.async.bulk.tensor.2d.shared::cluster.global.mbarrier::complete_tx::bytes [%0], [%1, {%3, %4}], [%2];"
      ::"r"(smem_u32(smem)), "l"(reinterpret_cast<uint64_t>(m)), "r"(smem_u32(bar)), "r"(c0), "r"(c1)
      : "memory");
}
__device__ __forceinline__ void tma_load_3d(void* smem, const CUtensorMap* m, uint64_t* bar, int c0, int c1,
                                            int c2) {
  asm volatile(
      "cp.async.bulk.tensor.3d.shared::cluster.global.mbarrier::complete_tx::bytes [%0], [%1, {%3, %4, %5}], [%2];"
      ::"r"(smem_u32(smem)), "l"(reinterpret_cast<uint64_t>(m)), "r"(smem_u32(bar)), "r"(c0), "r"(c1), "r"(c2)
      : "memory");
}

__device__ __forceinline__ void tma_load_4d(void* smem, const CUtensorMap* m, uint64_t* bar, int c0, int c1, int c2,
                                            int c3) {
  asm volatile(
      "cp.async.bulk.tensor.4d.shared::cluster.global.mbarrier::complete_tx::bytes [%0], [%1, {%3, %4, %5, %6}], [%2];"
      ::"r"(smem_u32(smem)), "l"(reinterpret_cast<uint64_t>(m)), "r"(smem_u32(bar)), "r"(c0), "r"(c1), "r"(c2), "r"(c3)
      : "memory");
}

__device__ __forceinline__ void tmem_alloc(uint32_t* smem_dst, uint32_t ncols) {
  asm volatile("tcgen05.alloc.cta_group::1.sync.aligned.shared::cta.b32 [%0], %1;" ::"r"(smem_u32(smem_dst)),
               "r"(ncols)
               : "memory");
}
__device__ __forceinline__ void tmem_relinquish() {
  asm volatile("tcgen05.relinquish_alloc_permit.cta_group::1.sync.aligned;" ::: "memory");
}
__device__ __forceinline__ void tmem_dealloc(uint32_t taddr, uint32_t ncols) {
  asm volatile("tcgen05.dealloc.cta_group::1.sync.aligned.b32 %0, %1;" ::"r"(taddr), "r"(ncols) : "memory");
}
__device__ __forceinline__ void tc_fence_before() { asm volatile("tcgen05.fence::before_thread_sync;" ::: "memory"); }
__device__ __forceinline__ void tc_fence_after() { asm volatile("tcgen05.fence::after_thread_sync;" ::: "memory"); }

__device__ __forceinline__ void umma_f16_ss(uint32_t tmem_d, uint64_t desc_a, uint64_t desc_b, uint32_t idesc,
                                            uint32_t accumulate) {
  asm volatile(
      "{\n\t.reg .pred p;\n\t"
      "setp.ne.b32 p, %4, 0;\n\t"
      "tcgen05.mma.cta_group::1.kind::f16 [%0], %1, %2, %3, p;\n\t}"
      ::"r"(tmem_d), "l"(desc_a), "l"(desc_b), "r"(idesc), "r"(accumulate)
      : "memory");
}
__device__ __forceinline__ void umma_f16_ts(uint32_t tmem_d, uint32_t tmem_a, uint64_t desc_b, uint32_t idesc,
                                            uint32_t accumulate) {
  asm volatile(
      "{\n\t.reg .pred p;\n\t"
      "setp.ne.b32 p, %4, 0;\n\t"
      "tcgen05.mma.cta_group::1.kind::f16 [%0], [%1], %2, %3, p;\n\t}"
      ::"r"(tmem_d), "r"(tmem_a), "l"(desc_b), "r"(idesc), "r"(accumulate)
      : "memory");
}
__device__ __forceinline__ void umma_commit(uint64_t* bar) {
  asm volatile("tcgen05.commit.cta_group::1.mbarrier::arrive::one.shared::cluster.b64 [%0];" ::"r"(smem_u32(bar))
               : "memory");
}

__device__ __forceinline__ void tmem_ld_32x32(uint32_t taddr, uint32_t (&r)[32]) {
  asm volatile(
      "tcgen05.ld.sync.aligned.32x32b.x32.b32 "
      "{%0, %1, %2, %3, %4, %5, %6, %7, %8, %9, %10, %11, %12, %13, %14, %15, "
      "%16, %17, %18, %19, %20, %21, %22, %23, %24, %25, %26, %27, %28, %29, %30, %31}, [%32];"
      : "=r"(r[0]), "=r"(r[1]), "=r"(r[2]), "=r"(r[3]), "=r"(r[4]), "=r"(r[5]), "=r"(r[6]), "=r"(r[7]),
        "=r"(r[8]), "=r"(r[9]), "=r"(r[10]), "=r"(r[11]), "=r"(r[12]), "=r"(r[13]), "=r"(r[14]), "=r"(r[15]),
        "=r"(r[16]), "=r"(r[17]), "=r"(r[18]), "=r"(r[19]), "=r"(r[20]), "=r"(r[21]), "=r"(r[22]), "=r"(r[23]),
        "=r"(r[24]), "=r"(r[25]), "=r"(r[26]), "=r"(r[27]), "=r"(r[28]), "=r"(r[29]), "=r"(r[30]), "=r"(r[31])
      : "r"(taddr)
      : "memory");
}
__device__ __forceinline__ void tmem_ld_32x16(uint32_t taddr, uint32_t (&r)[16]) {
  asm volatile(
      "tcgen05.ld.sync.aligned.32x32b.x16.b32 "
      "{%0, %1, %2, %3, %4, %5, %6, %7, %8, %9, %10, %11, %12, %13, %14, %15}, [%16];"
      : "=r"(r[0]), "=r"(r[1]), "=r"(r[2]), "=r"(r[3]), "=r"(r[4]), "=r"(r[5]), "=r"(r[6]), "=r"(r[7]),
        "=r"(r[8]), "=r"(r[9]), "=r"(r[10]), "=r"(r[11]), "=r"(r[12]), "=r"(r[13]), "=r"(r[14]), "=r"(r[15])
      : "r"(taddr)
      : "memory");
}
__device__ __forceinline__ void tmem_ld_32x2(uint32_t taddr, uint32_t (&r)[2]) {
  asm volatile("tcgen05.ld.sync.aligned.32x32b.x2.b32 {%0, %1}, [%2];" : "=r"(r[0]), "=r"(r[1]) : "r"(taddr) : "memory");
}
__device__ __forceinline__ void tmem_ld_wait() { asm volatile("tcgen05.wait::ld.sync.aligned;" ::: "memory"); }
__device__ __forceinline__ void tmem_ld_wait16(uint32_t (&r)[16]) {
  asm volatile("tcgen05.wait::ld.sync.aligned;"
               : "+r"(r[0]), "+r"(r[1]), "+r"(r[2]), "+r"(r[3]), "+r"(r[4]), "+r"(r[5]), "+r"(r[6]), "+r"(r[7]),
                 "+r"(r[8]), "+r"(r[9]), "+r"(r[10]), "+r"(r[11]), "+r"(r[12]), "+r"(r[13]), "+r"(r[14]), "+r"(r[15])
               :
               : "memory");
}

__device__ __forceinline__ void tmem_st_32x16(uint32_t taddr, const uint32_t (&r)[16]) {
  asm volatile(
      "tcgen05.st.sync.aligned.32x32b.x16.b32 [%0], "
      "{%1, %2, %3, %4, %5, %6, %7, %8, %9, %10, %11, %12, %13, %14, %15, %16};"
      ::"r"(taddr), "r"(r[0]), "r"(r[1]), "r"(r[2]), "r"(r[3]), "r"(r[4]), "r"(r[5]), "r"(r[6]), "r"(r[7]),
      "r"(r[8]), "r"(r[9]), "r"(r[10]), "r"(r[11]), "r"(r[12]), "r"(r[13]), "r"(r[14]), "r"(r[15])
      : "memory");
}
__device__ __forceinline__ void tmem_st_32x8(uint32_t taddr, const uint32_t (&r)[8]) {
  asm volatile("tcgen05.st.sync.aligned.32x32b.x8.b32 [%0], {%1, %2, %3, %4, %5, %6, %7, %8};"
               ::"r"(taddr), "r"(r[0]), "r"(r[1]), "r"(r[2]), "r"(r[3]), "r"(r[4]), "r"(r[5]), "r"(r[6]), "r"(r[7])
               : "memory");
}
__device__ __forceinline__ void tmem_st_wait() { asm volatile("tcgen05.wait::st.sync.aligned;" ::: "memory"); }

__device__ __forceinline__ void sts128(uint32_t addr, uint32_t x, uint32_t y, uint32_t z, uint32_t w) {
  asm volatile("st.shared.v4.b32 [%0], {%1, %2, %3, %4};" ::"r"(addr), "r"(x), "r"(y), "r"(z), "r"(w) : "memory");
}
__device__ __forceinline__ ulonglong2 lds128_b64x2(uint32_t addr) {
  ulonglong2 v;
  asm volatile("ld.shared.v2.b64 {%0, %1}, [%2];" : "=l"(v.x), "=l"(v.y) : "r"(addr) : "memory");
  return v;
}

__device__ __forceinline__ void tma_store_4d(const CUtensorMap* tm, const void* smem_src, int c0, int c1, int c2, int c3) {
  asm volatile("cp.async.bulk.tensor.4d.global.shared::cta.bulk_group [%0, {%2, %3, %4, %5}], [%1];"
               ::"l"(reinterpret_cast<uint64_t>(tm)), "r"(smem_u32(smem_src)), "r"(c0), "r"(c1), "r"(c2), "r"(c3)
               : "memory");
}
__device__ __forceinline__ void tma_store_commit() { asm volatile("cp.async.bulk.commit_group;" ::: "memory"); }
__device__ __forceinline__ void tma_store_wait_read() { asm volatile("cp.async.bulk.wait_group.read 0;" ::: "memory"); }
__device__ __forceinline__ void tma_store_wait_all() { asm volatile("cp.async.bulk.wait_group 0;" ::: "memory"); }

__device__ __forceinline__ uint32_t cluster_ctarank() {
  uint32_t r;
  asm volatile("mov.u32 %0, %%cluster_ctarank;" : "=r"(r));
  return r;
}
__device__ __forceinline__ void cluster_sync_all() {
  asm volatile("barrier.cluster.arrive.release.aligned;" ::: "memory");
  asm volatile("barrier.cluster.wait.acquire.aligned;" ::: "memory");
}
constexpr uint32_t kPeerBitMask = 0xFEFFFFFF;
__device__ __forceinline__ void tma_load_2d_2sm(void* smem, const CUtensorMap* m, uint64_t* bar, int c0, int c1) {
  asm volatile(
      "cp.async.bulk.tensor.2d.cta_group::2.shared::cluster.global.mbarrier::complete_tx::bytes [%0], [%1, {%3, %4}], [%2];"
      ::"r"(smem_u32(smem)), "l"(reinterpret_cast<uint64_t>(m)), "r"(smem_u32(bar) & kPeerBitMask), "r"(c0), "r"(c1)
      : "memory");
}
__device__ __forceinline__ void tma_load_4d_2sm(void* smem, const CUtensorMap* m, uint64_t* bar, int c0, int c1, int c2,
                                                int c3) {
  asm volatile(
      "cp.async.bulk.tensor.4d.cta_group::2.shared::cluster.global.mbarrier::complete_tx::bytes [%0], [%1, {%3, %4, %5, %6}], [%2];"
      ::"r"(smem_u32(smem)), "l"(reinterpret_cast<uint64_t>(m)), "r"(smem_u32(bar) & kPeerBitMask), "r"(c0), "r"(c1),
      "r"(c2), "r"(c3)
      : "memory");
}
__device__ __forceinline__ void tmem_alloc_2sm(uint32_t* smem_dst, uint32_t ncols) {
  asm volatile("tcgen05.alloc.cta_group::2.sync.aligned.shared::cta.b32 [%0], %1;" ::"r"(smem_u32(smem_dst)),
               "r"(ncols)
               : "memory");
}
__device__ __forceinline__ void tmem_relinquish_2sm() {
  asm volatile("tcgen05.relinquish_alloc_permit.cta_group::2.sync.aligned;" ::: "memory");
}
__device__ __forceinline__ void tmem_dealloc_2sm(uint32_t taddr, uint32_t ncols) {
  asm volatile("tcgen05.dealloc.cta_group::2.sync.aligned.b32 %0, %1;" ::"r"(taddr), "r"(ncols) : "memory");
}
__device__ __forceinline__ void umma_f16_ss_2sm(uint32_t tmem_d, uint64_t desc_a, uint64_t desc_b, uint32_t idesc,
                                                uint32_t accumulate) {
  asm volatile(
      "{\n\t.reg .pred p;\n\t"
      "setp.ne.b32 p, %4, 0;\n\t"
      "tcgen05.mma.cta_group::2.kind::f16 [%0], %1, %2, %3, p;\n\t}"
      ::"r"(tmem_d), "l"(desc_a), "l"(desc_b), "r"(idesc), "r"(accumulate)
      : "memory");
}
__device__ __forceinline__ void umma_commit_2sm(uint64_t* bar) {
  asm volatile(
      "tcgen05.commit.cta_group::2.mbarrier::arrive::one.shared::cluster.multicast::cluster.b64 [%0], %1;"
      ::"r"(smem_u32(bar)), "h"(static_cast<uint16_t>(3))
      : "memory");
}
__device__ __forceinline__ void mbar_arrive_remote(uint64_t* bar, uint32_t cta) {
  asm volatile(
      "{\n\t.reg .b32 ra;\n\t"
      "mapa.shared::cluster.u32 ra, %0, %1;\n\t"
      "mbarrier.arrive.shared::cluster.b64 _, [ra];\n\t}"
      ::"r"(smem_u32(bar)), "r"(cta)
      : "memory");
}

__device__ __forceinline__ void mbar_arrive_remote_cluster(uint64_t* bar, uint32_t cta) {
  asm volatile(
      "{\n\t.reg .b32 ra;\n\t"
      "mapa.shared::cluster.u32 ra, %0, %1;\n\t"
      "mbarrier.arrive.release.cluster.shared::cluster.b64 _, [ra];\n\t}"
      ::"r"(smem_u32(bar)), "r"(cta)
      : "memory");
}
__device__ __forceinline__ void mbar_wait_cluster(uint64_t* bar, uint32_t parity) {
  uint32_t ok;
  do {
    asm volatile(
        "{\n\t.reg .pred P;\n\t"
        "mbarrier.try_wait.parity.acquire.cluster.shared::cta.b64 P, [%1], %2, %3;\n\t"
        "selp.u32 %0, 1, 0, P;\n\t}"
        : "=r"(ok)
        : "r"(smem_u32(bar)), "r"(parity), "r"(kMbarSuspendHintNs)
        : "memory");
  } while (!ok);
}

__device__ __forceinline__ uint64_t make_desc_kmajor_sw128(uint32_t smem_addr) {
  uint64_t d = 0;
  d |= static_cast<uint64_t>((smem_addr >> 4) & 0x3FFF);
  d |= static_cast<uint64_t>(1) << 16;
  d |= static_cast<uint64_t>(1024 >> 4) << 32;
  d |= static_cast<uint64_t>(1) << 46;
  d |= static_cast<uint64_t>(2) << 61;
  return d;
}

__host__ __device__ constexpr uint32_t make_idesc_f16(int M, int N, bool bf16, bool b_mn_major = false) {
  return (1u << 4) | ((bf16 ? 1u : 0u) << 7) | ((bf16 ? 1u : 0u) << 10) | ((b_mn_major ? 1u : 0u) << 16) |
         (static_cast<uint32_t>(N >> 3) << 17) | (static_cast<uint32_t>(M >> 4) << 24);
}

}
```

### friendly-stable-audio-tools_b200/csrc/runtime.cu

```cuda
#include <mutex>

#include "common.cuh"
#include "gemm.cuh"
#include "kernels.h"
#include <cstdlib>

namespace satb {

static thread_local std::string g_last_error;
unsigned long long g_launch_count = 0;

void set_last_error(const std::string& msg) { g_last_error = msg; }
const char* get_last_error() { return g_last_error.c_str(); }

bool gemm_use_2cta() {
  static int v = -1;
  if (v < 0) {
    const char* e = getenv("SATB_GEMM");
    v = (e && std::string(e) == "1cta") ? 0 : 1;
  }
  return v == 1;
}

bool ln_fold_enabled() {
  static int v = -1;
  if (v < 0) {
    const char* e = getenv("SATB_LN");
    v = (e && std::string(e) == "fold") ? 1 : 0;
  }
  return v == 1;
}

bool raw_stream_16bit() {
  static int v = -1;
  if (v < 0) {
    const char* e = getenv("SATB_RAW");
    v = (e && std::string(e) == "fp32") ? 0 : 1;
  }
  return v == 1;
}

bool conv_halo_enabled() {
  static int v = -1;
  if (v < 0) {
    const char* e = getenv("SATB_CONV_HALO");
    v = (e && std::string(e) == "off") ? 0 : 1;
  }
  return v == 1;
}

bool conv_epi_masked() {
  static int v = -1;
  if (v < 0) {
    const char* e = getenv("SATB_CONV_EPI");
    v = (e && std::string(e) == "general") ? 0 : 1;
  }
  return v == 1;
}

bool resunit_use_fused() {
  static int v = -1;
  if (v < 0) {
    const char* e = getenv("SATB_RESUNIT");
    v = (e && std::string(e) == "unfused") ? 0 : 1;
  }
  return v == 1;
}

int device_sm_count() {
  static int cached[64] = {};
  int dev = 0;
  cudaGetDevice(&dev);
  if (dev < 0 || dev >= 64) dev = 0;
  if (cached[dev] == 0) {
    cudaDeviceGetAttribute(&cached[dev], cudaDevAttrMultiProcessorCount, dev);
    if (cached[dev] <= 0) cached[dev] = 148;
  }
  return cached[dev];
}

typedef CUresult (*EncodeTiledFn)(CUtensorMap*, CUtensorMapDataType, cuuint32_t, void*, const cuuint64_t*,
                                  const cuuint64_t*, const cuuint32_t*, const cuuint32_t*, CUtensorMapInterleave,
                                  CUtensorMapSwizzle, CUtensorMapL2promotion, CUtensorMapFloatOOBfill);

static EncodeTiledFn get_encode_fn() {
  static EncodeTiledFn fn = nullptr;
  static std::once_flag once;
  std::call_once(once, [] {
    void* p = nullptr;
    cudaDriverEntryPointQueryResult qres;
    if (cudaGetDriverEntryPoint("cuTensorMapEncodeTiled", &p, cudaEnableDefault, &qres) == cudaSuccess &&
        qres == cudaDriverEntryPointSuccess)
      fn = reinterpret_cast<EncodeTiledFn>(p);
  });
  return fn;
}

int make_tmap_a(CUtensorMap* m, const void* ptr, int K, int L, int batches, int64_t row_stride_elems,
                int64_t batch_stride_elems, int stride, int box_rows) {
  EncodeTiledFn fn = get_encode_fn();
  SATB_REQUIRE(fn != nullptr, "cuTensorMapEncodeTiled entry point unavailable");
  SATB_REQUIRE((reinterpret_cast<uintptr_t>(ptr) & 15) == 0, "TMA base must be 16B aligned");
  SATB_REQUIRE((row_stride_elems * 2) % 16 == 0 && (batch_stride_elems * 2) % 16 == 0, "TMA strides must be 16B multiples");
  cuuint64_t dims[4] = {static_cast<cuuint64_t>(K), static_cast<cuuint64_t>(stride), static_cast<cuuint64_t>(L),
                        static_cast<cuuint64_t>(batches)};
  cuuint64_t strides[3] = {static_cast<cuuint64_t>(row_stride_elems) * 2,
                           static_cast<cuuint64_t>(row_stride_elems) * 2 * stride,
                           static_cast<cuuint64_t>(batch_stride_elems) * 2};
  cuuint32_t box[4] = {static_cast<cuuint32_t>(kBlockK), 1, static_cast<cuuint32_t>(box_rows), 1};
  cuuint32_t estr[4] = {1, 1, 1, 1};
  CUresult r = fn(m, CU_TENSOR_MAP_DATA_TYPE_UINT16, 4, const_cast<void*>(ptr), dims, strides, box, estr,
                  CU_TENSOR_MAP_INTERLEAVE_NONE, CU_TENSOR_MAP_SWIZZLE_128B, CU_TENSOR_MAP_L2_PROMOTION_L2_256B,
                  CU_TENSOR_MAP_FLOAT_OOB_FILL_NONE);
  if (r != CUDA_SUCCESS) {
    set_last_error("cuTensorMapEncodeTiled(A) failed with CUresult " + std::to_string(static_cast<int>(r)) +
                   " K=" + std::to_string(K) + " L=" + std::to_string(L) + " batches=" + std::to_string(batches) +
                   " rs=" + std::to_string(row_stride_elems) + " bs=" + std::to_string(batch_stride_elems));
    return -3;
  }
  return 0;
}

int make_tmap_b(CUtensorMap* m, const void* ptr, int K, int rows, int64_t row_stride_elems, int box_rows) {
  EncodeTiledFn fn = get_encode_fn();
  SATB_REQUIRE(fn != nullptr, "cuTensorMapEncodeTiled entry point unavailable");
  SATB_REQUIRE((reinterpret_cast<uintptr_t>(ptr) & 15) == 0, "TMA base must be 16B aligned");
  SATB_REQUIRE((row_stride_elems * 2) % 16 == 0, "TMA strides must be 16B multiples");
  cuuint64_t dims[2] = {static_cast<cuuint64_t>(K), static_cast<cuuint64_t>(rows)};
  cuuint64_t strides[1] = {static_cast<cuuint64_t>(row_stride_elems) * 2};
  cuuint32_t box[2] = {static_cast<cuuint32_t>(kBlockK), static_cast<cuuint32_t>(box_rows)};
  cuuint32_t estr[2] = {1, 1};
  CUresult r = fn(m, CU_TENSOR_MAP_DATA_TYPE_UINT16, 2, const_cast<void*>(ptr), dims, strides, box, estr,
                  CU_TENSOR_MAP_INTERLEAVE_NONE, CU_TENSOR_MAP_SWIZZLE_128B, CU_TENSOR_MAP_L2_PROMOTION_L2_256B,
                  CU_TENSOR_MAP_FLOAT_OOB_FILL_NONE);
  if (r != CUDA_SUCCESS) {
    set_last_error("cuTensorMapEncodeTiled(B) failed with CUresult " + std::to_string(static_cast<int>(r)) +
                   " K=" + std::to_string(K) + " rows=" + std::to_string(rows));
    return -3;
  }
  return 0;
}

}
```

### friendly-stable-audio-tools_b200/stable_audio_tools/_native.py

```python
import ctypes
import os

import torch

_HERE = os.path.dirname(os.path.abspath(__file__))
LIB_PATH = os.path.join(os.path.dirname(_HERE), "libsatb200.so")

_lib = None


class NativeError(RuntimeError):
    pass


class SatbDitConfig(ctypes.Structure):
    _fields_ = [(n, ctypes.c_int) for n in (
        "io_channels", "embed_dim", "depth", "num_heads", "cond_token_dim", "global_cond_dim",
        "project_cond_tokens", "project_global_cond", "global_cond_type", "patch_size", "operand_dtype", "qk_norm",
        "input_concat_dim", "prepend_cond_dim")]


SATB_MAX_STAGES = 8


class SatbOobleckConfig(ctypes.Structure):
    _fields_ = [("in_channels", ctypes.c_int), ("channels", ctypes.c_int), ("latent_dim", ctypes.c_int),
                ("n_stages", ctypes.c_int), ("c_mults", ctypes.c_int * SATB_MAX_STAGES),
                ("strides", ctypes.c_int * SATB_MAX_STAGES), ("final_tanh", ctypes.c_int),
                ("is_decoder", ctypes.c_int), ("operand_dtype", ctypes.c_int)]


_VP, _I, _LL, _F = ctypes.c_void_p, ctypes.c_int, ctypes.c_longlong, ctypes.c_float
SIGNATURES = {
    "satb_last_error": (ctypes.c_char_p, []),
    "satb_abi_version": (_I, []),
    "satb_launch_count": (ctypes.c_ulonglong, []),
    "satb_reset_launch_count": (None, []),
    "satb_add_launch_count": (None, [ctypes.c_ulonglong]),
    "satb_dit_create": (_I, [ctypes.POINTER(SatbDitConfig), ctypes.POINTER(_VP)]),
    "satb_dit_destroy": (None, [_VP]),
    "satb_dit_load_weight": (_I, [_VP, ctypes.c_char_p, _VP, _LL, _VP]),
    "satb_dit_finalize": (_I, [_VP, _VP]),
    "satb_dit_reserve": (_I, [_VP, _I, _I]),
    "satb_dit_set_prepend_cond": (_I, [_VP, _VP, _I, _I, _VP]),
    "satb_dit_prepare_cond": (_I, [_VP, _VP, _VP, _VP, _I, _I, _I, _VP]),
    "satb_dit_forward": (_I, [_VP, _VP, _VP, _VP, _I, _I, _F, _F, _VP]),
    "satb_dit_forward_debug": (_I, [_VP, _VP, _VP, _VP, _VP, _I, _I, _F, _F, _VP]),
    "satb_dit_profile": (_I, [_VP, _I]),
    "satb_dit_profile_read": (_I, [_VP, _VP, _VP]),
    "satb_snake_beta": (_I, [_VP, _VP, _VP, _VP, _I, _I, _LL, _I, _VP]),
    "satb_sampler_update": (_I, [_VP, _VP, _VP, _VP, _VP, _VP, _VP, _VP, _LL] + [_F] * 8 + [_VP]),
    "satb_layernorm": (_I, [_VP, _VP, _VP, _VP, _I, _I, _I, _VP]),
    "satb_linear_f32out": (_I, [_VP, _VP, _VP, _I, _I, _I, _I, _VP]),
    "satb_attention": (_I, [_VP, _VP, _VP, _VP, _I, _I, _I, _I, _I, _I, _VP]),
    "satb_debug_attention_occupancy": (_I, [_I, _I]),
    "satb_attention_trace": (_I, [_VP, _VP, _VP, _VP, _I, _I, _I, _I, _I, _I, _VP, _VP]),
    "satb_oobleck_create": (_I, [ctypes.POINTER(SatbOobleckConfig), ctypes.POINTER(_VP)]),
    "satb_oobleck_destroy": (None, [_VP]),
    "satb_oobleck_load_weight": (_I, [_VP, ctypes.c_char_p, _VP, _LL, _VP]),
    "satb_oobleck_finalize": (_I, [_VP, _VP]),
    "satb_oobleck_decode": (_I, [_VP, _VP, _VP, _I, _I, _VP]),
    "satb_oobleck_encode": (_I, [_VP, _VP, _VP, _I, _LL, _VP]),
}


def lib():
    global _lib
    if _lib is None:
        if not os.path.exists(LIB_PATH):
            raise NativeError(
                f"{LIB_PATH} not found: build it with `python friendly-stable-audio-tools_b200/build.py` "
                "(or __graft_entry__.build()); this package has no non-CUDA fallback")
        l = ctypes.CDLL(LIB_PATH)
        for name, (res, args) in SIGNATURES.items():
            fn = getattr(l, name)
            fn.restype = res
            fn.argtypes = args
        _lib = l
    return _lib


def check(rc):
    if rc != 0:
        msg = lib().satb_last_error()
        raise NativeError(f"satb200 error {rc}: {msg.decode() if msg else '?'}")


def stream_ptr(device=None):
    return ctypes.c_void_p(torch.cuda.current_stream(device).cuda_stream)


def dev_f32(t, name="tensor"):
    if not isinstance(t, torch.Tensor) or not t.is_cuda:
        raise NativeError(f"{name} must be a CUDA tensor: this package runs on the GPU only (no CPU fallback)")
    if t.dtype != torch.float32 or not t.is_contiguous():
        raise NativeError(f"{name} must be contiguous float32")
    return ctypes.c_void_p(t.data_ptr())


def ptr(t):
    return ctypes.c_void_p(t.data_ptr()) if t is not None else None


def launch_count():
    return int(lib().satb_launch_count())
```

### include/satb200.h

```cpp
#ifndef SATB200_H_
#define SATB200_H_

#ifdef __cplusplus
extern "C" {
#endif

#define SATB_ABI_VERSION 3

typedef struct SatbDit SatbDit;
typedef struct SatbOobleck SatbOobleck;

typedef struct SatbDitConfig {
  int io_channels;
  int embed_dim;
  int depth;
  int num_heads;
  int cond_token_dim;
  int global_cond_dim;
  int project_cond_tokens;
  int project_global_cond;
  int global_cond_type;
  int patch_size;
  int operand_dtype;
  int qk_norm;
  int input_concat_dim;
  int prepend_cond_dim;
} SatbDitConfig;

#define SATB_MAX_STAGES 8
typedef struct SatbOobleckConfig {
  int in_channels;
  int channels;
  int latent_dim;
  int n_stages;
  int c_mults[SATB_MAX_STAGES];
  int strides[SATB_MAX_STAGES];
  int final_tanh;
  int is_decoder;
  int operand_dtype;
} SatbOobleckConfig;

const char* satb_last_error(void);
int satb_abi_version(void);
unsigned long long satb_launch_count(void);
void satb_reset_launch_count(void);
void satb_add_launch_count(unsigned long long n);

int satb_dit_create(const SatbDitConfig* cfg, SatbDit** out);
void satb_dit_destroy(SatbDit* h);
int satb_dit_load_weight(SatbDit* h, const char* name, const float* src, long long numel, void* stream);
int satb_dit_finalize(SatbDit* h, void* stream);
int satb_dit_reserve(SatbDit* h, int rows, int L);
int satb_dit_set_prepend_cond(SatbDit* h, const float* prepend, int B, int n_tokens, void* stream);
int satb_dit_prepare_cond(SatbDit* h, const float* cross, const float* neg_cross, const float* global, int B,
                          int Mctx, int use_cfg, void* stream);
int satb_dit_forward(SatbDit* h, const float* x, const float* t, float* out, int B, int L, float cfg_scale,
                     float scale_phi, void* stream);
int satb_dit_forward_debug(SatbDit* h, const float* x, const float* t, float* out, float* hidden, int B, int L,
                           float cfg_scale, float scale_phi, void* stream);

int satb_dit_profile(SatbDit* h, int enable);
int satb_dit_profile_read(SatbDit* h, float* ms, int* count);

int satb_snake_beta(const float* x, const float* alpha, const float* beta, float* y, int B, int C, long long T,
                    int logscale, void* stream);
int satb_layernorm(const float* x, const float* gamma, const float* beta, void* out16, int rows, int D, int bf16,
                   void* stream);
int satb_linear_f32out(const void* a16, const void* w16, float* c, int M, int N, int K, int bf16, void* stream);
int satb_sampler_update(const float* x, const float* v, const float* den_1, const float* den_2, const float* noise,
                        float* den, float* x_next, float* x_in_next, long long n, float c_skip, float c_out, float a,
                        float b, float c, float d, float s, float c_in_next, void* stream);
int satb_attention(const void* q16, const void* k16, const void* v16, void* o16, int B, int H, int Hkv, int Nq, int Nk,
                   int bf16, void* stream);

int satb_debug_attention_occupancy(int dyn_smem, int carveout_pct);
int satb_attention_trace(const void* q16, const void* k16, const void* v16, void* o16, int B, int H, int Hkv, int Nq,
                         int Nk, int bf16, unsigned long long* dbg, void* stream);

int satb_oobleck_create(const SatbOobleckConfig* cfg, SatbOobleck** out);
void satb_oobleck_destroy(SatbOobleck* h);
int satb_oobleck_load_weight(SatbOobleck* h, const char* name, const float* src, long long numel, void* stream);
int satb_oobleck_finalize(SatbOobleck* h, void* stream);
int satb_oobleck_decode(SatbOobleck* h, const float* z, float* audio, int B, int L, void* stream);
int satb_oobleck_encode(SatbOobleck* h, const float* audio, float* latents, int B, long long T, void* stream);

#ifdef __cplusplus
}
#endif
#endif
```

Before: 50.67.

## Add stream-K scheduling for the FF2 GEMM in the 2-CTA tcgen05 kernel

Adds a stream-K hybrid schedule to the 2-CTA GEMM. When the tile count leaves a partial last wave and K is long, the remaining tiles plus one wave are split across cluster pairs by K-block ranges. Partial accumulators are spilled to a global workspace and handed between pairs through release/acquire flags, then restored into TMEM before the epilogue. It is enabled only for the FF2 projection, which has a large K, and is meant to remove wave-quantization idle time. The cost is extra workspace traffic, cross-CTA flag waits, and more complex kernel control flow.

```diff
diff --git a/friendly-stable-audio-tools_b200/csrc/api.cu b/friendly-stable-audio-tools_b200/csrc/api.cu
--- a/friendly-stable-audio-tools_b200/csrc/api.cu
+++ b/friendly-stable-audio-tools_b200/csrc/api.cu
@@ -44,6 +44,24 @@
   return bf16 ? launch_gemm<EpiStore32, 64, true>(ta, tb, s, ep, st) : launch_gemm<EpiStore32, 64, false>(ta, tb, s, ep, st);
 }
 
+int satb_gemm_plan(int total_tiles, int num_kb, int pairs, int* sk_tiles, int* out, int cap) {
+  SATB_REQUIRE(total_tiles >= 0 && num_kb >= 1 && pairs >= 1 && sk_tiles && out, "bad argument");
+  *sk_tiles = gemm_sk_tiles(total_tiles, num_kb, pairs);
+  int n = 0;
+  for (int p = 0; p < pairs; ++p) {
+    const PairWork w = pair_work(total_tiles, num_kb, pairs, *sk_tiles, p);
+    for (int i = 0; i < w.n_items; ++i, ++n) {
+      if (n >= cap) return -1;
+      const Piece pc = pair_piece(w, num_kb, pairs, p, i);
+      out[4 * n] = p;
+      out[4 * n + 1] = pc.tile;
+      out[4 * n + 2] = pc.kb0;
+      out[4 * n + 3] = pc.kb1;
+    }
+  }
+  return n;
+}
+
 int satb_sampler_update(const float* x, const float* v, const float* den_1, const float* den_2, const float* noise,
                         float* den, float* x_next, float* x_in_next, long long n, float c_skip, float c_out, float a,
                         float b, float c, float d, float s, float c_in_next, void* stream) {
diff --git a/friendly-stable-audio-tools_b200/csrc/dit.cu b/friendly-stable-audio-tools_b200/csrc/dit.cu
--- a/friendly-stable-audio-tools_b200/csrc/dit.cu
+++ b/friendly-stable-audio-tools_b200/csrc/dit.cu
@@ -66,8 +66,8 @@
   }
 };
 
-template <class Epi, int BN, bool BF16>
-static int linear(TmapCache& tc, const void* A, int64_t lda, int M, int K, const void* W, int N,
+template <class Epi, int BN, bool BF16, bool SK = false>
+static int linear(TmapCache& tc, const StreamKWs* sk, const void* A, int64_t lda, int M, int K, const void* W, int N,
                   const typename Epi::Params& ep, cudaStream_t stream) {
   const CUtensorMap *ta, *tb;
   SATB_PROPAGATE(tc.get_a(A, K, M, 1, lda, static_cast<int64_t>(M) * lda, &ta));
@@ -77,23 +77,23 @@
   if constexpr (BN == 256 || BN == 128) {
     if (gemm_use_2cta() && M >= 1024) {
       SATB_PROPAGATE(tc.get_b(W, K, N, K, BN / 2, &tb));
-      return launch_gemm_2cta<Epi, BN, BF16>(*ta, *tb, s, ep, stream);
+      return launch_gemm_2cta<Epi, BN, BF16, SK>(*ta, *tb, s, ep, stream, nullptr, sk);
     }
   }
   SATB_PROPAGATE(tc.get_b(W, K, N, K, BN, &tb));
   return launch_gemm<Epi, BN, BF16>(*ta, *tb, s, ep, stream);
 }
 
-template <class Epi, bool BF16>
-static int linear_auto(TmapCache& tc, const void* A, int64_t lda, int M, int K, const void* W, int N,
+template <class Epi, bool BF16, bool SK = false>
+static int linear_auto(TmapCache& tc, const StreamKWs* sk, const void* A, int64_t lda, int M, int K, const void* W, int N,
                        const typename Epi::Params& ep, cudaStream_t stream) {
   const double sms = device_sm_count();
   auto eff = [&](int bn) {
     const double waves = static_cast<double>(ceil_div(M, kBlockM)) * ceil_div(N, bn) / sms;
     return waves / std::ceil(waves);
   };
-  if (N % 128 == 0 && eff(128) * 0.9 > eff(256)) return linear<Epi, 128, BF16>(tc, A, lda, M, K, W, N, ep, stream);
-  return linear<Epi, 256, BF16>(tc, A, lda, M, K, W, N, ep, stream);
+  if (N % 128 == 0 && eff(128) * 0.9 > eff(256)) return linear<Epi, 128, BF16, SK>(tc, sk, A, lda, M, K, W, N, ep, stream);
+  return linear<Epi, 256, BF16, SK>(tc, sk, A, lda, M, K, W, N, ep, stream);
 }
 
 struct LayerW {
@@ -133,6 +133,8 @@
   bool cfg_on = false, has_cross = false, has_global = false;
   TmapCache tmaps;
   DevBuf ws_h, ws_a16, ws_qkv, ws_attn, ws_q16, ws_ff, ws_ain, ws_y, ws_small, ws_cond, ws_kv, ws_rope, ws_stats;
+  DevBuf ws_sk;
+  StreamKWs sk;
   int rope_len = 0;
   int res_R = 0, res_L = 0, res_P = -1;
   bool prof_on = false;
@@ -225,7 +227,7 @@
   for (void* p : d->owned) cudaFree(p);
   d->ws_h.release(); d->ws_a16.release(); d->ws_qkv.release(); d->ws_attn.release(); d->ws_q16.release();
   d->ws_ff.release(); d->ws_ain.release(); d->ws_y.release(); d->ws_small.release(); d->ws_cond.release();
-  d->ws_kv.release(); d->ws_rope.release(); d->ws_stats.release(); d->ws_prep.release();
+  d->ws_kv.release(); d->ws_rope.release(); d->ws_stats.release(); d->ws_prep.release(); d->ws_sk.release();
   delete d;
 }
 
@@ -427,6 +429,14 @@
   SATB_PROPAGATE(d->ws_ain.ensure(M * d->Cin * 2));
   SATB_PROPAGATE(d->ws_y.ensure(M * d->C * 4));
   SATB_PROPAGATE(d->ws_stats.ensure(3 * M * kLnSlots * sizeof(float2)));
+  if (!d->ws_sk.p) {
+    const size_t pairs = device_sm_count() / 2;
+    const size_t ws_bytes = pairs * kSkWsFloatsPerPair * sizeof(float);
+    SATB_PROPAGATE(d->ws_sk.ensure(ws_bytes + pairs * 2 * kEpiWarps * sizeof(uint32_t)));
+    SATB_CHECK_CUDA(cudaMemset(d->ws_sk.as<uint8_t>() + ws_bytes, 0, pairs * 2 * kEpiWarps * sizeof(uint32_t)));
+    d->sk.ws = d->ws_sk.as<float>();
+    d->sk.flags = reinterpret_cast<uint32_t*>(d->ws_sk.as<uint8_t>() + ws_bytes);
+  }
   SATB_PROPAGATE(ensure_rope(d, N_seq));
   d->tmaps.maps.clear();
   d->res_R = R;
@@ -512,30 +522,30 @@
     const int Mr = static_cast<int>(rows);
     if (d->bf16) {
       typedef EpiStore16<true> E;
-      SATB_PROPAGATE((linear<E, 128, true>(d->tmaps, in16, d->ct, Mr, d->ct, d->ce0_w, d->ce, E::Params{mid16, d->ce, nullptr, 1}, st)));
-      SATB_PROPAGATE((linear<E, 128, true>(d->tmaps, mid16, d->ce, Mr, d->ce, d->ce2_w, d->ce, E::Params{ce16, d->ce, nullptr, 0}, st)));
+      SATB_PROPAGATE((linear<E, 128, true>(d->tmaps, &d->sk, in16, d->ct, Mr, d->ct, d->ce0_w, d->ce, E::Params{mid16, d->ce, nullptr, 1}, st)));
+      SATB_PROPAGATE((linear<E, 128, true>(d->tmaps, &d->sk, mid16, d->ce, Mr, d->ce, d->ce2_w, d->ce, E::Params{ce16, d->ce, nullptr, 0}, st)));
       for (int i = 0; i < d->depth; ++i) {
         uint16_t* kv = d->ws_kv.as<uint16_t>() + static_cast<size_t>(i) * rows * 2 * d->ce;
         if (d->qk_norm) {
           typedef EpiHeadNorm16<true> EN;
-          SATB_PROPAGATE((linear<EN, 128, true>(d->tmaps, ce16, d->ce, Mr, d->ce, d->layers[i].w_kv, 2 * d->ce,
+          SATB_PROPAGATE((linear<EN, 128, true>(d->tmaps, &d->sk, ce16, d->ce, Mr, d->ce, d->layers[i].w_kv, 2 * d->ce,
                                                  EN::Params{kv, 2 * d->ce, d->ce, 0, 1, nullptr, nullptr}, st)));
         } else {
-          SATB_PROPAGATE((linear<E, 128, true>(d->tmaps, ce16, d->ce, Mr, d->ce, d->layers[i].w_kv, 2 * d->ce, E::Params{kv, 2 * d->ce, nullptr, 0}, st)));
+          SATB_PROPAGATE((linear<E, 128, true>(d->tmaps, &d->sk, ce16, d->ce, Mr, d->ce, d->layers[i].w_kv, 2 * d->ce, E::Params{kv, 2 * d->ce, nullptr, 0}, st)));
         }
       }
     } else {
       typedef EpiStore16<false> E;
-      SATB_PROPAGATE((linear<E, 128, false>(d->tmaps, in16, d->ct, Mr, d->ct, d->ce0_w, d->ce, E::Params{mid16, d->ce, nullptr, 1}, st)));
-      SATB_PROPAGATE((linear<E, 128, false>(d->tmaps, mid16, d->ce, Mr, d->ce, d->ce2_w, d->ce, E::Params{ce16, d->ce, nullptr, 0}, st)));
+      SATB_PROPAGATE((linear<E, 128, false>(d->tmaps, &d->sk, in16, d->ct, Mr, d->ct, d->ce0_w, d->ce, E::Params{mid16, d->ce, nullptr, 1}, st)));
+      SATB_PROPAGATE((linear<E, 128, false>(d->tmaps, &d->sk, mid16, d->ce, Mr, d->ce, d->ce2_w, d->ce, E::Params{ce16, d->ce, nullptr, 0}, st)));
       for (int i = 0; i < d->depth; ++i) {
         uint16_t* kv = d->ws_kv.as<uint16_t>() + static_cast<size_t>(i) * rows * 2 * d->ce;
         if (d->qk_norm) {
           typedef EpiHeadNorm16<false> EN;
-          SATB_PROPAGATE((linear<EN, 128, false>(d->tmaps, ce16, d->ce, Mr, d->ce, d->layers[i].w_kv, 2 * d->ce,
+          SATB_PROPAGATE((linear<EN, 128, false>(d->tmaps, &d->sk, ce16, d->ce, Mr, d->ce, d->layers[i].w_kv, 2 * d->ce,
                                                  EN::Params{kv, 2 * d->ce, d->ce, 0, 1, nullptr, nullptr}, st)));
         } else {
-          SATB_PROPAGATE((linear<E, 128, false>(d->tmaps, ce16, d->ce, Mr, d->ce, d->layers[i].w_kv, 2 * d->ce, E::Params{kv, 2 * d->ce, nullptr, 0}, st)));
+          SATB_PROPAGATE((linear<E, 128, false>(d->tmaps, &d->sk, ce16, d->ce, Mr, d->ce, d->layers[i].w_kv, 2 * d->ce, E::Params{kv, 2 * d->ce, nullptr, 0}, st)));
         }
       }
     }
@@ -581,7 +591,7 @@
   SATB_PROPAGATE(launch_skinny_linear(sw.te_h, d->te2_w, d->te2_b, d->has_global ? sw.ge : nullptr, sw.tok, B, D, D,
                                       d->adaln ? 1 : 0, st));
   SATB_PROPAGATE(launch_dit_pre(x, ain, R, B, d->Cin, L, P, BF16, st));
-  SATB_PROPAGATE((linear<EpiStore32, 256, BF16>(d->tmaps, ain, d->Cin, M, d->Cin, d->w_in16, D, EpiStore32::Params{h, D, nullptr}, st)));
+  SATB_PROPAGATE((linear<EpiStore32, 256, BF16>(d->tmaps, &d->sk, ain, d->Cin, M, d->Cin, d->w_in16, D, EpiStore32::Params{h, D, nullptr}, st)));
   const int64_t ssg_ld = static_cast<int64_t>(d->depth) * 6 * D;
   if (P > 0) {
     SATB_PROPAGATE(launch_write_prepend(sw.tok, d->Pp > 0 ? d->ws_prep.as<float>() : nullptr, h, R, B, N_seq, D, d->Pp, st));
@@ -610,16 +620,16 @@
       if (d->qk_norm) {
         typedef EpiHeadNorm16<BF16> E;
         typename E::Params ep{qkv, 3 * D, 2 * D, 2 * D, N_seq, cos_tab, sin_tab};
-        SATB_PROPAGATE((linear<E, 256, BF16>(d->tmaps, a16, D, M, D, W.w_qkv, 3 * D, ep, st)));
+        SATB_PROPAGATE((linear<E, 256, BF16>(d->tmaps, &d->sk, a16, D, M, D, W.w_qkv, 3 * D, ep, st)));
       } else {
         if (fused && i > 0) {
           typedef EpiQkvRope<BF16, true> E;
           typename E::Params ep{qkv, 3 * D, 2 * D, N_seq, cos_tab, sin_tab, fold(S1, W.c_qkv, W.d_qkv)};
-          SATB_PROPAGATE((linear<E, 256, BF16>(d->tmaps, a16, D, M, D, W.w_qkv, 3 * D, ep, st)));
+          SATB_PROPAGATE((linear<E, 256, BF16>(d->tmaps, &d->sk, a16, D, M, D, W.w_qkv, 3 * D, ep, st)));
         } else {
           typedef EpiQkvRope<BF16> E;
           typename E::Params ep{qkv, 3 * D, 2 * D, N_seq, cos_tab, sin_tab, no_ln};
-          SATB_PROPAGATE((linear<E, 256, BF16>(d->tmaps, a16, D, M, D, W.w_qkv, 3 * D, ep, st)));
+          SATB_PROPAGATE((linear<E, 256, BF16>(d->tmaps, &d->sk, a16, D, M, D, W.w_qkv, 3 * D, ep, st)));
         }
       }
     }
@@ -635,10 +645,10 @@
       if (fused) {
         typedef EpiResidualLN<BF16> E;
         typename E::Params ep{h, D, nullptr, a16, W.ca_g, W.ff_g, S2, S3, Mc};
-        SATB_PROPAGATE((linear<E, 256, BF16>(d->tmaps, att, D, M, D, W.w_o, D, ep, st)));
+        SATB_PROPAGATE((linear<E, 256, BF16>(d->tmaps, &d->sk, att, D, M, D, W.w_o, D, ep, st)));
       } else {
         EpiResidual::Params ep{h, D, nullptr, ssg_l ? ssg_l + 2 * D : nullptr, N_seq, static_cast<int>(ssg_ld), B};
-        SATB_PROPAGATE((linear_auto<EpiResidual, BF16>(d->tmaps, att, D, M, D, W.w_o, D, ep, st)));
+        SATB_PROPAGATE((linear_auto<EpiResidual, BF16>(d->tmaps, &d->sk, att, D, M, D, W.w_o, D, ep, st)));
       }
     }
     if (Mc > 0) {
@@ -648,16 +658,16 @@
       if (d->qk_norm) {
         typedef EpiHeadNorm16<BF16> E;
         typename E::Params ep{q16, D, D, 0, N_seq, nullptr, nullptr};
-        SATB_PROPAGATE((linear_auto<E, BF16>(d->tmaps, a16, D, Mc, D, W.w_q, D, ep, st)));
+        SATB_PROPAGATE((linear_auto<E, BF16>(d->tmaps, &d->sk, a16, D, Mc, D, W.w_q, D, ep, st)));
       } else {
         if (fused) {
           typedef EpiStore16<BF16, true> E;
           typename E::Params ep{q16, D, nullptr, 0, fold(S2, W.c_q, W.d_q)};
-          SATB_PROPAGATE((linear_auto<E, BF16>(d->tmaps, a16, D, Mc, D, W.w_q, D, ep, st)));
+          SATB_PROPAGATE((linear_auto<E, BF16>(d->tmaps, &d->sk, a16, D, Mc, D, W.w_q, D, ep, st)));
         } else {
           typedef EpiStore16<BF16> E;
           typename E::Params ep{q16, D, nullptr, 0, no_ln};
-          SATB_PROPAGATE((linear_auto<E, BF16>(d->tmaps, a16, D, Mc, D, W.w_q, D, ep, st)));
+          SATB_PROPAGATE((linear_auto<E, BF16>(d->tmaps, &d->sk, a16, D, Mc, D, W.w_q, D, ep, st)));
         }
       }
       const uint16_t* kv = d->ws_kv.as<uint16_t>() + static_cast<size_t>(i) * d->Rc * d->Mctx * 2 * d->ce;
@@ -668,10 +678,10 @@
       if (fused) {
         typedef EpiResidualLN<BF16> E;
         typename E::Params ep{h, D, nullptr, a16, W.ff_g, W.ff_g, S3, S3, Mc};
-        SATB_PROPAGATE((linear<E, 256, BF16>(d->tmaps, att, D, Mc, D, W.w_co, D, ep, st)));
+        SATB_PROPAGATE((linear<E, 256, BF16>(d->tmaps, &d->sk, att, D, Mc, D, W.w_co, D, ep, st)));
       } else {
         EpiResidual::Params ep{h, D, nullptr, nullptr, N_seq, 0, 1};
-        SATB_PROPAGATE((linear_auto<EpiResidual, BF16>(d->tmaps, att, D, Mc, D, W.w_co, D, ep, st)));
+        SATB_PROPAGATE((linear_auto<EpiResidual, BF16>(d->tmaps, &d->sk, att, D, Mc, D, W.w_co, D, ep, st)));
       }
     }
     if (!fused) {
@@ -684,11 +694,11 @@
       if (fused) {
         typedef EpiSwiglu<BF16, true> E;
         typename E::Params ep{ff, d->ffi, W.b_ff1, fold(S3, W.c_ff1, W.d_ff1)};
-        SATB_PROPAGATE((linear<E, 256, BF16>(d->tmaps, a16, D, M, D, W.w_ff1, 2 * d->ffi, ep, st)));
+        SATB_PROPAGATE((linear<E, 256, BF16>(d->tmaps, &d->sk, a16, D, M, D, W.w_ff1, 2 * d->ffi, ep, st)));
       } else {
         typedef EpiSwiglu<BF16> E;
         typename E::Params ep{ff, d->ffi, W.b_ff1, no_ln};
-        SATB_PROPAGATE((linear<E, 256, BF16>(d->tmaps, a16, D, M, D, W.w_ff1, 2 * d->ffi, ep, st)));
+        SATB_PROPAGATE((linear<E, 256, BF16>(d->tmaps, &d->sk, a16, D, M, D, W.w_ff1, 2 * d->ffi, ep, st)));
       }
     }
     {
@@ -697,17 +707,17 @@
         const bool last = i + 1 == d->depth;
         typedef EpiResidualLN<BF16> E;
         typename E::Params ep{h, D, W.b_ff2, a16, last ? nullptr : d->layers[i + 1].pre_g, nullptr, last ? nullptr : S1, nullptr, M};
-        SATB_PROPAGATE((linear<E, 256, BF16>(d->tmaps, ff, d->ffi, M, d->ffi, W.w_ff2, D, ep, st)));
+        SATB_PROPAGATE((linear<E, 256, BF16, true>(d->tmaps, &d->sk, ff, d->ffi, M, d->ffi, W.w_ff2, D, ep, st)));
       } else {
         EpiResidual::Params ep{h, D, W.b_ff2, ssg_l ? ssg_l + 5 * D : nullptr, N_seq, static_cast<int>(ssg_ld), B};
-        SATB_PROPAGATE((linear_auto<EpiResidual, BF16>(d->tmaps, ff, d->ffi, M, d->ffi, W.w_ff2, D, ep, st)));
+        SATB_PROPAGATE((linear_auto<EpiResidual, BF16, true>(d->tmaps, &d->sk, ff, d->ffi, M, d->ffi, W.w_ff2, D, ep, st)));
       }
     }
   }
   if (hidden_out)
     SATB_CHECK_CUDA(cudaMemcpyAsync(hidden_out, h, static_cast<size_t>(M) * D * 4, cudaMemcpyDeviceToDevice, st));
   if (!fused || d->depth == 0) SATB_PROPAGATE(launch_cast_rows(h, a16, nullptr, M, D, D, D, BF16, st));
-  SATB_PROPAGATE((linear<EpiStore32, 64, BF16>(d->tmaps, a16, D, M, D, d->w_out16, C, EpiStore32::Params{y, C, nullptr}, st)));
+  SATB_PROPAGATE((linear<EpiStore32, 64, BF16>(d->tmaps, &d->sk, a16, D, M, D, d->w_out16, C, EpiStore32::Params{y, C, nullptr}, st)));
   SATB_PROPAGATE(launch_dit_post(y, out, B, C, L, N_seq, P, d->cfg_on ? 1 : 0, cfg_scale, scale_phi, st));
   return 0;
 }
diff --git a/friendly-stable-audio-tools_b200/csrc/gemm.cuh b/friendly-stable-audio-tools_b200/csrc/gemm.cuh
--- a/friendly-stable-audio-tools_b200/csrc/gemm.cuh
+++ b/friendly-stable-audio-tools_b200/csrc/gemm.cuh
@@ -291,6 +291,52 @@
   }
 }
 
+struct StreamKWs {
+  float* ws = nullptr;
+  uint32_t* flags = nullptr;
+};
+constexpr int kSkWsFloatsPerPair = 2 * kEpiWarps * 16 * 256;
+struct GemmPlan {
+  int sk_tiles = 0;
+  StreamKWs w;
+};
+struct PairWork {
+  int n_items, n_dp, n_full, has_pre, has_suf;
+  int dp_tiles, tb, kbb, te, kbe, full_first;
+};
+struct Piece {
+  int tile, kb0, kb1;
+};
+__host__ __device__ __forceinline__ PairWork pair_work(int total_tiles, int num_kb, int pairs, int sk_tiles, int p) {
+  PairWork w{};
+  w.dp_tiles = total_tiles - sk_tiles;
+  w.n_dp = p < w.dp_tiles ? (w.dp_tiles - 1 - p) / pairs + 1 : 0;
+  if (sk_tiles > 0) {
+    const long long iters = static_cast<long long>(sk_tiles) * num_kb;
+    const int b = static_cast<int>(p * iters / pairs), e = static_cast<int>((p + 1) * iters / pairs);
+    w.tb = b / num_kb;
+    w.kbb = b - w.tb * num_kb;
+    w.te = e / num_kb;
+    w.kbe = e - w.te * num_kb;
+    w.has_pre = w.kbe != 0;
+    w.has_suf = w.kbb != 0;
+    w.full_first = w.tb + w.has_suf;
+    w.n_full = w.te - w.full_first;
+  }
+  w.n_items = w.has_pre + w.n_dp + w.n_full + w.has_suf;
+  return w;
+}
+__host__ __device__ __forceinline__ Piece pair_piece(const PairWork& w, int num_kb, int pairs, int p, int i) {
+  if (i < w.has_pre) return Piece{w.dp_tiles + w.te, 0, w.kbe};
+  i -= w.has_pre;
+  if (i < w.n_dp) return Piece{p + i * pairs, 0, num_kb};
+  i -= w.n_dp;
+  if (i < w.n_full) return Piece{w.dp_tiles + w.full_first + i, 0, num_kb};
+  return Piece{w.dp_tiles + w.tb, w.kbb, num_kb};
+}
+int gemm_sk_tiles(int total_tiles, int num_kb, int pairs);
+inline int num_kb_of(const GemmShape& s) { return (s.K + kBlockK - 1) / kBlockK * s.n_taps * s.n_parts; }
+
 template <int BN, int kEpiStage = 0>
 struct Gemm2Cfg {
   static constexpr int kStageA = kBlockM * kBlockK * 2;
@@ -303,10 +349,11 @@
   static_assert(BN == 256 || BN == 128, "BN must be 128/256");
 };
 
-template <class Epi, int BN, bool BF16>
+template <class Epi, int BN, bool BF16, bool SK = false>
 __global__ void __cluster_dims__(2, 1, 1) __launch_bounds__(kGemmThreads, 1)
 gemm_tcgen05_2cta_kernel(const __grid_constant__ CUtensorMap tmA, const __grid_constant__ CUtensorMap tmB,
-                         const __grid_constant__ CUtensorMap tmA2, const GemmShape s, const typename Epi::Params ep) {
+                         const __grid_constant__ CUtensorMap tmA2, const GemmShape s, const typename Epi::Params ep,
+                         const GemmPlan plan) {
   using Cfg = Gemm2Cfg<BN, Epi::kStageBytes>;
   extern __shared__ uint8_t smem_raw[];
   uint8_t* smem = reinterpret_cast<uint8_t*>((reinterpret_cast<uintptr_t>(smem_raw) + 1023) & ~uintptr_t(1023));
@@ -315,7 +362,10 @@
   uint64_t* empty_bar = bars + Cfg::kStages;
   uint64_t* tfull_bar = bars + 2 * Cfg::kStages;
   uint64_t* tempty_bar = tfull_bar + 2;
-  uint32_t* tmem_slot = reinterpret_cast<uint32_t*>(tempty_bar + 2);
+  uint64_t* restore_bar = tempty_bar + 2;
+  PairWork* work_s = reinterpret_cast<PairWork*>(restore_bar + 1);
+  uint32_t* tmem_slot = reinterpret_cast<uint32_t*>(work_s + 1);
+  static_assert((2 * Cfg::kStages + 5) * sizeof(uint64_t) + sizeof(PairWork) + sizeof(uint32_t) <= 256, "barrier area");
 
   const int warp = threadIdx.x >> 5;
   const int lane = threadIdx.x & 31;
@@ -341,7 +391,9 @@
       mbar_init(&tfull_bar[i], 1);
       mbar_init(&tempty_bar[i], 16);
     }
+    mbar_init(restore_bar, 16);
     fence_mbar_init();
+    if constexpr (SK) *work_s = pair_work(total_tiles, num_kb, n_clusters, plan.sk_tiles, cluster_id);
   }
   cluster_sync_all();
   if (warp == 2) {
@@ -352,35 +404,39 @@
   __syncthreads();
   tc_fence_after();
   const uint32_t tmem_base = *tmem_slot;
+  const PairWork& work = *work_s;
   pdl_launch_dependents();
   if (warp != 0) pdl_wait();
 
   if (warp == 0) {
     if (elect_one()) {
       int pre = 0;
-      if (s.b_static && cluster_id < total_tiles) {
-        pre = num_kb < Cfg::kStages ? num_kb : Cfg::kStages;
-        const int n0 = (cluster_id / tiles_per_n) * BN + rank * (BN / 2);
-        for (int kb = 0; kb < pre; ++kb) {
+      if (s.b_static && (SK ? work.n_items > 0 : cluster_id < total_tiles)) {
+        const Piece pc = SK ? pair_piece(work, num_kb, n_clusters, cluster_id, 0) : Piece{cluster_id, 0, num_kb};
+        pre = pc.kb1 - pc.kb0 < Cfg::kStages ? pc.kb1 - pc.kb0 : Cfg::kStages;
+        const int n0 = (pc.tile / tiles_per_n) * BN + rank * (BN / 2);
+        for (int j = 0; j < pre; ++j) {
+          const int kb = pc.kb0 + j;
           const int pidx = kb / kb_per_part, kbp = kb - pidx * kb_per_part;
           const int part = split_part(pidx, s.n_parts);
           const int tap = kbp / kb_per_tap;
           const int k0 = (kbp - tap * kb_per_tap) * kBlockK;
-          if (rank == 0) mbar_expect_tx(&full_bar[kb], 2 * Cfg::kStage);
-          tma_load_2d_2sm(smem + kb * Cfg::kStage + Cfg::kStageA, &tmB, &full_bar[kb], k0,
+          if (rank == 0) mbar_expect_tx(&full_bar[j], 2 * Cfg::kStage);
+          tma_load_2d_2sm(smem + j * Cfg::kStage + Cfg::kStageA, &tmB, &full_bar[j], k0,
                           tap * s.b_tap_rows + n0 + (part == 2 ? s.b_part_rows : 0));
         }
       }
       pdl_wait();
       int stage = 0;
       uint32_t phase = 0;
-      for (int tile = cluster_id; tile < total_tiles; tile += n_clusters) {
-        const int nt = tile / tiles_per_n;
-        const int rem = tile - nt * tiles_per_n;
+      for (int item = 0, tile = cluster_id; SK ? item < work.n_items : tile < total_tiles; ++item, tile += n_clusters) {
+        const Piece pc = SK ? pair_piece(work, num_kb, n_clusters, cluster_id, item) : Piece{tile, 0, num_kb};
+        const int nt = pc.tile / tiles_per_n;
+        const int rem = pc.tile - nt * tiles_per_n;
         const int batch = rem / m_tiles;
         const int m0 = (rem - batch * m_tiles) * 2 * kBlockM + rank * kBlockM;
         const int n0 = nt * BN + rank * (BN / 2);
-        for (int kb = 0; kb < num_kb; ++kb) {
+        for (int kb = pc.kb0; kb < pc.kb1; ++kb) {
           const int pidx = kb / kb_per_part, kbp = kb - pidx * kb_per_part;
           const int part = split_part(pidx, s.n_parts);
           const int tap = kbp / kb_per_tap;
@@ -388,7 +444,7 @@
           mbar_wait(&empty_bar[stage], phase ^ 1);
           uint8_t* sa = smem + stage * Cfg::kStage;
           uint8_t* sb = sa + Cfg::kStageA;
-          const bool b_done = tile == cluster_id && kb < pre;
+          const bool b_done = (SK ? item == 0 : tile == cluster_id) && kb - pc.kb0 < pre;
           if (rank == 0 && !b_done) mbar_expect_tx(&full_bar[stage], 2 * Cfg::kStage);
           const int u = s.tap_base + tap * s.tap_step;
           int ph = 0, ro = u;
@@ -413,11 +469,13 @@
       uint32_t phase = 0;
       int acc = 0;
       uint32_t acc_phase = 0;
-      for (int tile = cluster_id; tile < total_tiles; tile += n_clusters) {
+      for (int item = 0, tile = cluster_id; SK ? item < work.n_items : tile < total_tiles; ++item, tile += n_clusters) {
+        const Piece pc = SK ? pair_piece(work, num_kb, n_clusters, cluster_id, item) : Piece{tile, 0, num_kb};
         mbar_wait(&tempty_bar[acc], acc_phase ^ 1);
+        if (pc.kb0 > 0) mbar_wait_cluster(restore_bar, 0);
         tc_fence_after();
         const uint32_t d_tmem = tmem_base + acc * BN;
-        for (int kb = 0; kb < num_kb; ++kb) {
+        for (int kb = pc.kb0; kb < pc.kb1; ++kb) {
           mbar_wait(&full_bar[stage], phase);
           tc_fence_after();
           const uint32_t a_addr = smem_u32(smem + stage * Cfg::kStage);
@@ -445,16 +503,68 @@
     const int q = warp & 3;
     const int half = (warp - 4) >> 2;
     constexpr int kChunks = BN / Epi::kCols;
+    constexpr int kGroups = BN / 64, kGroupsPerChunk = Epi::kCols / 32;
+    auto group_col = [&](int g) { return ((g / kGroupsPerChunk) * 2 + half) * Epi::kCols + (g % kGroupsPerChunk) * 32; };
+    auto wslot = [&]() { return (cluster_id * 2 + static_cast<int>(rank)) * kEpiWarps + (warp - 4); };
+    auto ws_part = [&](int slot) { return reinterpret_cast<float4*>(plan.w.ws) + static_cast<size_t>(slot) * 4 * BN + lane; };
+    auto restore = [&](int buf) {
+      const int slot = wslot() - 2 * kEpiWarps;
+      if (lane == 0) {
+        while (ld_acquire_gpu(plan.w.flags + slot) == 0) {
+        }
+      }
+      __syncwarp();
+      const float4* src = ws_part(slot);
+      const uint32_t t_row = tmem_base + (static_cast<uint32_t>(q * 32) << 16) + buf * BN;
+#pragma unroll 1
+      for (int g = 0; g < kGroups; ++g) {
+        uint32_t r[32];
+#pragma unroll
+        for (int v = 0; v < 8; ++v) {
+          const float4 x = __ldcg(src + (g * 8 + v) * 32);
+          r[4 * v] = __float_as_uint(x.x); r[4 * v + 1] = __float_as_uint(x.y);
+          r[4 * v + 2] = __float_as_uint(x.z); r[4 * v + 3] = __float_as_uint(x.w);
+        }
+        tmem_st_32x32(t_row + group_col(g), r);
+      }
+      tmem_st_wait();
+      __syncwarp();
+      if (lane == 0) st_relaxed_gpu(plan.w.flags + slot, 0);
+      tc_fence_before();
+      if (lane == 0) mbar_arrive_remote_cluster(restore_bar, 0);
+    };
     int acc = 0;
     uint32_t acc_phase = 0;
-    for (int tile = cluster_id; tile < total_tiles; tile += n_clusters) {
-      const int nt = tile / tiles_per_n;
-      const int rem = tile - nt * tiles_per_n;
+    for (int item = 0, tile = cluster_id; SK ? item < work.n_items : tile < total_tiles; ++item, tile += n_clusters) {
+      const Piece pc = SK ? pair_piece(work, num_kb, n_clusters, cluster_id, item) : Piece{tile, 0, num_kb};
+      const int nt = pc.tile / tiles_per_n;
+      const int rem = pc.tile - nt * tiles_per_n;
       const int batch = rem / m_tiles;
       const int m0 = (rem - batch * m_tiles) * 2 * kBlockM + rank * kBlockM;
       const int n0 = nt * BN;
       mbar_wait(&tfull_bar[acc], acc_phase);
       tc_fence_after();
+      if (pc.kb1 < num_kb) {
+        float4* dst = ws_part(wslot());
+        const uint32_t t_row = tmem_base + (static_cast<uint32_t>(q * 32) << 16) + acc * BN;
+#pragma unroll 1
+        for (int g = 0; g < kGroups; ++g) {
+          uint32_t r[32];
+          tmem_ld_32x32(t_row + group_col(g), r);
+          tmem_ld_wait();
+#pragma unroll
+          for (int v = 0; v < 8; ++v)
+            __stcg(dst + (g * 8 + v) * 32, make_float4(__uint_as_float(r[4 * v]), __uint_as_float(r[4 * v + 1]),
+                                                       __uint_as_float(r[4 * v + 2]), __uint_as_float(r[4 * v + 3])));
+        }
+        __threadfence();
+        tc_fence_before();
+        __syncwarp();
+        if (lane == 0) {
+          mbar_arrive_remote(&tempty_bar[acc], 0);
+          st_release_gpu(plan.w.flags + wslot(), 1);
+        }
+      } else {
       EpiCtx c;
       c.l = m0 + q * 32 + lane;
       c.batch = batch;
@@ -503,6 +613,9 @@
       tc_fence_before();
       __syncwarp();
       if (lane == 0) mbar_arrive_remote(&tempty_bar[acc], 0);
+      }
+      if constexpr (SK)
+        if (work.has_suf && item == (work.n_items >= 3 ? work.n_items - 3 : 0)) restore((work.n_items - 1) & 1);
       if (++acc == 2) {
         acc = 0;
         acc_phase ^= 1;
@@ -1320,11 +1433,11 @@
   return 0;
 }
 
-template <class Epi, int BN, bool BF16>
+template <class Epi, int BN, bool BF16, bool SK = false>
 int launch_gemm_2cta(const CUtensorMap& tmA, const CUtensorMap& tmB, const GemmShape& s, const typename Epi::Params& ep,
-                     cudaStream_t stream, const CUtensorMap* tmA2 = nullptr) {
+                     cudaStream_t stream, const CUtensorMap* tmA2 = nullptr, const StreamKWs* sk = nullptr) {
   using Cfg = Gemm2Cfg<BN, Epi::kStageBytes>;
-  auto kern = gemm_tcgen05_2cta_kernel<Epi, BN, BF16>;
+  auto kern = gemm_tcgen05_2cta_kernel<Epi, BN, BF16, SK>;
   static PerDeviceOnce attr;
   if (attr.first()) SATB_CHECK_CUDA(cudaFuncSetAttribute(kern, cudaFuncAttributeMaxDynamicSharedMemorySize, Cfg::kSmemBytes));
   const int m_tiles = ceil_div(s.L, 2 * kBlockM), n_tiles = ceil_div(s.N, BN);
@@ -1333,8 +1446,13 @@
   int clusters = device_sm_count() / 2;
   if (clusters > total) clusters = total;
   SATB_REQUIRE(s.n_parts == 1 || tmA2 != nullptr, "split-operand GEMM needs the second A tensor map");
+  GemmPlan plan;
+  if (SK && sk && sk->ws && s.n_taps == 1 && s.n_parts == 1) {
+    plan.sk_tiles = gemm_sk_tiles(total, num_kb_of(s), clusters);
+    plan.w = *sk;
+  }
   SATB_CHECK_CUDA(launch_pdl(kern, dim3(2 * clusters), dim3(kGemmThreads), Cfg::kSmemBytes, stream, tmA, tmB,
-                             tmA2 ? *tmA2 : tmA, s, ep));
+                             tmA2 ? *tmA2 : tmA, s, ep, plan));
   count_launch();
   return 0;
 }
diff --git a/friendly-stable-audio-tools_b200/csrc/kernels.h b/friendly-stable-audio-tools_b200/csrc/kernels.h
--- a/friendly-stable-audio-tools_b200/csrc/kernels.h
+++ b/friendly-stable-audio-tools_b200/csrc/kernels.h
@@ -13,6 +13,7 @@
 bool conv_epi_masked();
 bool resunit_use_fused();
 bool gemm_use_2cta();
+bool gemm_stream_k();
 bool ln_fold_enabled();
 bool raw_stream_16bit();
 
diff --git a/friendly-stable-audio-tools_b200/csrc/ptx.cuh b/friendly-stable-audio-tools_b200/csrc/ptx.cuh
--- a/friendly-stable-audio-tools_b200/csrc/ptx.cuh
+++ b/friendly-stable-audio-tools_b200/csrc/ptx.cuh
@@ -175,7 +175,30 @@
                ::"r"(taddr), "r"(r[0]), "r"(r[1]), "r"(r[2]), "r"(r[3]), "r"(r[4]), "r"(r[5]), "r"(r[6]), "r"(r[7])
                : "memory");
 }
+__device__ __forceinline__ void tmem_st_32x32(uint32_t taddr, const uint32_t (&r)[32]) {
+  asm volatile(
+      "tcgen05.st.sync.aligned.32x32b.x32.b32 [%0], "
+      "{%1, %2, %3, %4, %5, %6, %7, %8, %9, %10, %11, %12, %13, %14, %15, %16, "
+      "%17, %18, %19, %20, %21, %22, %23, %24, %25, %26, %27, %28, %29, %30, %31, %32};"
+      ::"r"(taddr), "r"(r[0]), "r"(r[1]), "r"(r[2]), "r"(r[3]), "r"(r[4]), "r"(r[5]), "r"(r[6]), "r"(r[7]),
+      "r"(r[8]), "r"(r[9]), "r"(r[10]), "r"(r[11]), "r"(r[12]), "r"(r[13]), "r"(r[14]), "r"(r[15]),
+      "r"(r[16]), "r"(r[17]), "r"(r[18]), "r"(r[19]), "r"(r[20]), "r"(r[21]), "r"(r[22]), "r"(r[23]),
+      "r"(r[24]), "r"(r[25]), "r"(r[26]), "r"(r[27]), "r"(r[28]), "r"(r[29]), "r"(r[30]), "r"(r[31])
+      : "memory");
+}
 __device__ __forceinline__ void tmem_st_wait() { asm volatile("tcgen05.wait::st.sync.aligned;" ::: "memory"); }
+
+__device__ __forceinline__ uint32_t ld_acquire_gpu(const uint32_t* p) {
+  uint32_t v;
+  asm volatile("ld.acquire.gpu.global.u32 %0, [%1];" : "=r"(v) : "l"(p) : "memory");
+  return v;
+}
+__device__ __forceinline__ void st_release_gpu(uint32_t* p, uint32_t v) {
+  asm volatile("st.release.gpu.global.u32 [%0], %1;" ::"l"(p), "r"(v) : "memory");
+}
+__device__ __forceinline__ void st_relaxed_gpu(uint32_t* p, uint32_t v) {
+  asm volatile("st.relaxed.gpu.global.u32 [%0], %1;" ::"l"(p), "r"(v) : "memory");
+}
 
 __device__ __forceinline__ void sts128(uint32_t addr, uint32_t x, uint32_t y, uint32_t z, uint32_t w) {
   asm volatile("st.shared.v4.b32 [%0], {%1, %2, %3, %4};" ::"r"(addr), "r"(x), "r"(y), "r"(z), "r"(w) : "memory");
diff --git a/friendly-stable-audio-tools_b200/csrc/runtime.cu b/friendly-stable-audio-tools_b200/csrc/runtime.cu
--- a/friendly-stable-audio-tools_b200/csrc/runtime.cu
+++ b/friendly-stable-audio-tools_b200/csrc/runtime.cu
@@ -20,6 +20,22 @@
     v = (e && std::string(e) == "1cta") ? 0 : 1;
   }
   return v == 1;
+}
+
+bool gemm_stream_k() {
+  static int v = -1;
+  if (v < 0) {
+    const char* e = getenv("SATB_GEMM_SCHED");
+    v = (e && std::string(e) == "tiles") ? 0 : 1;
+  }
+  return v == 1;
+}
+
+constexpr int kSkMinKBlocks = 64;
+int gemm_sk_tiles(int total_tiles, int num_kb, int pairs) {
+  const int r = total_tiles % pairs;
+  if (!gemm_stream_k() || total_tiles < pairs || r == 0 || num_kb < kSkMinKBlocks) return 0;
+  return pairs + r;
 }
 
 bool ln_fold_enabled() {
diff --git a/friendly-stable-audio-tools_b200/stable_audio_tools/_native.py b/friendly-stable-audio-tools_b200/stable_audio_tools/_native.py
--- a/friendly-stable-audio-tools_b200/stable_audio_tools/_native.py
+++ b/friendly-stable-audio-tools_b200/stable_audio_tools/_native.py
@@ -52,6 +52,7 @@
     "satb_sampler_update": (_I, [_VP, _VP, _VP, _VP, _VP, _VP, _VP, _VP, _LL] + [_F] * 8 + [_VP]),
     "satb_layernorm": (_I, [_VP, _VP, _VP, _VP, _I, _I, _I, _VP]),
     "satb_linear_f32out": (_I, [_VP, _VP, _VP, _I, _I, _I, _I, _VP]),
+    "satb_gemm_plan": (_I, [_I, _I, _I, _VP, _VP, _I]),
     "satb_attention": (_I, [_VP, _VP, _VP, _VP, _I, _I, _I, _I, _I, _I, _VP]),
     "satb_debug_attention_occupancy": (_I, [_I, _I]),
     "satb_attention_trace": (_I, [_VP, _VP, _VP, _VP, _I, _I, _I, _I, _I, _I, _VP, _VP]),
diff --git a/include/satb200.h b/include/satb200.h
--- a/include/satb200.h
+++ b/include/satb200.h
@@ -67,6 +67,7 @@
 int satb_layernorm(const float* x, const float* gamma, const float* beta, void* out16, int rows, int D, int bf16,
                    void* stream);
 int satb_linear_f32out(const void* a16, const void* w16, float* c, int M, int N, int K, int bf16, void* stream);
+int satb_gemm_plan(int total_tiles, int num_kb, int pairs, int* sk_tiles, int* out, int cap);
 int satb_sampler_update(const float* x, const float* v, const float* den_1, const float* den_2, const float* noise,
                         float* den, float* x_next, float* x_in_next, long long n, float c_skip, float c_out, float a,
                         float b, float c, float d, float s, float c_in_next, void* stream);
```

Result: no change. 49.99, median of 6 (-1.3%).
